# vvvwo/KSS-ICP

Measured on AMD Instinct MI355X. Metric: icp_iterations_per_sec, higher is better.
Workload: dtype f32; 1 GPU; C2: one 100000x100000 uniform-sphere pair per GPU, 50 fixed ICP iterations + fitness pass per step (exact NN + cov reduce + host 3x3 SVD), R_z(10deg), jitter 1e-3; n_src=100000, n_tgt=100000, pairs_per_gpu=1, nn_engine=cell list + brute-force fallback, nn_arithmetic=reference (no fma)

## Files before the change

kss-icp_amd/csrc/kss_api.hip:

```cpp
#pragma clang fp contract(off)

#include <cmath>

#include "kss_ctx.hpp"
#include "kss_gicp.hpp"
#include "kss_robust.hpp"

extern "C" {

int kss_version(void) { return KSS_VERSION; }

const char* kss_status_string(int s) {
    switch (s) {
        case KSS_OK: return "ok";
        case KSS_ERR_ARG: return "invalid argument";
        case KSS_ERR_HIP: return "HIP runtime error";
        case KSS_ERR_NOMEM: return "out of memory";
        case KSS_ERR_NODEVICE: return "no usable GPU device";
        case KSS_ERR_CAPACITY: return "output buffer too small";
        case KSS_ERR_RCCL: return "RCCL error";
        case KSS_ERR_DEGENERATE: return "degenerate point-to-plane system";
        default: return "unknown status";
    }
}

const char* kss_last_error(const kss_ctx* ctx) { return ctx ? ctx->err.c_str() : ""; }

static int ctx_create_common(int device_id, void* stream, bool borrow, kss_ctx** out) {
    if (!out) return KSS_ERR_ARG;
    *out = nullptr;
    int n = 0;
    if (hipGetDeviceCount(&n) != hipSuccess || n <= 0) return KSS_ERR_NODEVICE;
    if (device_id < 0 || device_id >= n) return KSS_ERR_ARG;
    if (hipSetDevice(device_id) != hipSuccess) return KSS_ERR_NODEVICE;
    kss_ctx* c = new (std::nothrow) kss_ctx();
    if (!c) return KSS_ERR_NOMEM;
    c->device = device_id;
    if (borrow) {
        c->stream = (hipStream_t)stream;
        c->own_stream = false;
    } else {
        if (hipStreamCreateWithFlags(&c->stream, hipStreamNonBlocking) != hipSuccess) { delete c; return KSS_ERR_HIP; }
        c->own_stream = true;
    }
    kss_live_contexts().fetch_add(1);
    static std::atomic<unsigned long long> ctx_serial{0};
    c->seq = (ctx_serial.fetch_add(1) + 1ull) << 40;
    *out = c;
    return KSS_OK;
}

int kss_ctx_create(int device_id, kss_ctx** out) { return ctx_create_common(device_id, nullptr, false, out); }
int kss_ctx_create_on_stream(int device_id, void* hip_stream, kss_ctx** out) {
    return ctx_create_common(device_id, hip_stream, true, out);
}

int kss_ctx_destroy(kss_ctx* c) {
    if (!c) return KSS_ERR_ARG;
    hipSetDevice(c->device);
    hipStreamSynchronize(c->stream);
    prof_collect(c);
    for (auto& ep : c->ev_pool) { hipEventDestroy(ep.a); hipEventDestroy(ep.b); }
    c->ev_pool.clear();
    DevBuf* bufs[] = {&c->tgt4, &c->src0, &c->cur[0], &c->cur[1], &c->keys, &c->partials, &c->sums, &c->nn_work,
                      &c->red_work, &c->pair_red, &c->state, &c->cs, &c->scratch_a, &c->scratch_b, &c->scratch_c,
                      &c->stage_src, &c->stage_tgt, &c->stage_idx, &c->stage_d2, &c->stage_out, &c->g_counts, &c->g_slot, &c->g_start,
                      &c->g_cursor, &c->g_bsums, &c->g_sorted, &c->g_list, &c->g_count, &c->g_bbox, &c->g_partials, &c->g_start2, &c->g_pairs, &c->g_stamps, &c->g_pos, &c->g_nnst, &c->res_pos, &c->res_wc, &c->res_perm, &c->pack_seg, &c->reg_s, &c->reg_t, &c->reg_p, &c->reg_all, &c->reg_f, &c->reg_g, &c->oct_pts, &c->oct_cen, &c->oct_a, &c->oct_b, &c->oct_tmp, &c->pre_partials, &c->pre_state, &c->g_rowpair, &c->g_gate, &c->p2l_idx, &c->p2l_d2, &c->p2l_perm, &c->p2l_rows, &c->p2l_nrm, &c->p2l_n64, &c->trim_rows, &c->trim_state, &c->rob_keys, &c->gicp_snrm, &c->pb_desc, &c->pb_rowpair, &c->pb_nrm, &c->pb_rscale, &c->pb_snrm, &c->pb_gicp, &c->o2o_table, &c->o2o_idx, &c->o2o_d2, &c->recip_sorted, &c->recip_box, &c->recip_grids, &c->gate_bar, &c->res_gate, &c->bar_state};
    for (DevBuf* b : bufs)
        if (b->p) hipFree(b->p);
    if (c->h_sums) hipHostFree(c->h_sums);
    if (c->h_seq) hipHostFree(c->h_seq);
    if (c->h_p2l) hipHostFree(c->h_p2l);
    if (c->h_gicp) hipHostFree(c->h_gicp);
    if (c->h_box) hipHostFree(c->h_box);
    if (c->h_xf) hipHostFree(c->h_xf);
    if (c->h_state) hipHostFree(c->h_state);
    for (kss_vmap* m : c->vmaps) { vmap_free(m->b); delete m; }
    c->vmaps.clear();
    for (kss_ctx* w : c->workers) kss_ctx_destroy(w);
    c->workers.clear();
    if (c->own_stream) hipStreamDestroy(c->stream);
    kss_live_contexts().fetch_sub(1);
    delete c;
    return KSS_OK;
}

int kss_ctx_synchronize(kss_ctx* c) {
    if (!c) return KSS_ERR_ARG;
    HIPCHK(c, hipStreamSynchronize(c->stream));
    return KSS_OK;
}

void* kss_ctx_stream(kss_ctx* c) { return c ? (void*)c->stream : nullptr; }

int kss_ctx_set_nn_mode(kss_ctx* c, int nn_mode) {
    if (!c || nn_mode < KSS_NN_AUTO || nn_mode > KSS_NN_GRID) return KSS_ERR_ARG;
    c->nn_mode = nn_mode;
    return KSS_OK;
}

int kss_profile_enable(kss_ctx* c, int on) {
    if (!c) return KSS_ERR_ARG;
    c->prof = on > 0 ? on : 0;
    for (int k = 0; k < KSS_K_COUNT; ++k) c->prof_tick[k] = 0;
    if (c->prof) {
        HIPCHK(c, hipSetDevice(c->device));
        while (c->ev_pool.size() < 4096) {
            kss_ctx::EvPair ep;
            if (hipEventCreate(&ep.a) != hipSuccess) break;
            if (hipEventCreate(&ep.b) != hipSuccess) { hipEventDestroy(ep.a); break; }
            c->ev_pool.push_back(ep);
        }
    }
    return KSS_OK;
}
int kss_grid_stats(kss_ctx* c, double out[8]) {
    if (!c || !out) return KSS_ERR_ARG;
    for (int k = 0; k < 8; ++k) out[k] = c->grid_stats[k];
    return KSS_OK;
}
int kss_debug_grid_evals(kss_ctx* c, double out[2]) {
    if (!c || !out) return KSS_ERR_ARG;
    out[0] = c->evals_sum; out[1] = c->evals_launches;
    c->evals_sum = 0.0; c->evals_launches = 0.0;
    return KSS_OK;
}

int kss_debug_grid_stamps(kss_ctx* c, unsigned long long* out, int64_t cap) {
    if (!c || !out) return KSS_ERR_ARG;
    if (c->stamps_nblk > 0 && c->g_stamps.p) {
        hipStreamSynchronize(c->stream);
        c->last_stamps.resize((size_t)c->stamps_nblk * 16);
        if (hipMemcpy(c->last_stamps.data(), (const unsigned long long*)c->g_stamps.p + (size_t)(c->stamps_seq & 1) * c->stamps_nblk * 16,
                      c->last_stamps.size() * sizeof(unsigned long long), hipMemcpyDeviceToHost) != hipSuccess) return KSS_ERR_HIP;
    }
    const int64_t n = std::min<int64_t>(cap, (int64_t)c->last_stamps.size());
    for (int64_t i = 0; i < n; ++i) out[i] = c->last_stamps[(size_t)i];
    return (int)n;
}
int kss_profile_reset(kss_ctx* c) {
    if (!c) return KSS_ERR_ARG;
    HIPCHK(c, hipStreamSynchronize(c->stream));
    prof_collect(c);
    for (int k = 0; k < KSS_K_COUNT; ++k) { c->prof_ms[k] = 0; c->prof_n[k] = 0; }
    return KSS_OK;
}
int kss_profile_event_overhead(kss_ctx* c, double* ms) {
    if (!c || !ms) return KSS_ERR_ARG;
    HIPCHK(c, hipSetDevice(c->device));
    hipEvent_t a = nullptr, b = nullptr;
    HIPCHK(c, hipEventCreate(&a));
    HIPCHK(c, hipEventCreate(&b));
    for (int i = 0; i < 16; ++i) launch_empty(c->stream);
    HIPCHK(c, hipStreamSynchronize(c->stream));
    double tot = 0.0;
    const int reps = 200;
    for (int i = 0; i < reps; ++i) {
        hipEventRecord(a, c->stream);
        launch_empty(c->stream);
        hipEventRecord(b, c->stream);
        HIPCHK(c, hipStreamSynchronize(c->stream));
        float e = 0.f;
        HIPCHK(c, hipEventElapsedTime(&e, a, b));
        tot += e;
    }
    hipEventDestroy(a);
    hipEventDestroy(b);
    *ms = tot / reps;
    return KSS_OK;
}
int kss_profile_get(kss_ctx* c, int k, double* total_ms, int64_t* launches) {
    if (!c || k < 0 || k >= KSS_K_COUNT) return KSS_ERR_ARG;
    HIPCHK(c, hipStreamSynchronize(c->stream));
    prof_collect(c);
    if (total_ms) *total_ms = c->prof_ms[k];
    if (launches) *launches = c->prof_n[k];
    return KSS_OK;
}

}

extern "C" {

int kss_icp_default_params(kss_icp_params* p) {
    if (!p) return KSS_ERR_ARG;
    std::memset(p, 0, sizeof *p);
    p->max_iterations = 1000;
    p->max_corr_dist = 1.0;
    p->transformation_epsilon = 1e-10;
    p->euclidean_fitness_epsilon = 0.001;
    p->abs_mse_epsilon = 1e-12;
    p->min_correspondences = 3;
    p->compute_fitness = 1;
    return KSS_OK;
}

int kss_icp_dev(kss_ctx* c, const float* d_src, int64_t ns, const float* d_tgt, int64_t nt,
                const kss_icp_params* p, kss_icp_result* res) {
    if (!c) return KSS_ERR_ARG;
    if (ns <= 0 || nt <= 0) return set_err(c, KSS_ERR_ARG, "icp: empty cloud");
    const int64_t so[2] = {0, ns}, to[2] = {0, nt};
    return icp_run_dev(c, d_src, so, d_tgt, to, 1, false, KSS_F32, p, res);
}

int kss_icp(kss_ctx* c, const float* src, int64_t ns, const float* tgt, int64_t nt,
            const kss_icp_params* p, kss_icp_result* res) {
    if (!c || !src || !tgt) return set_err(c, KSS_ERR_ARG, "icp: null cloud");
    if (ns <= 0 || nt <= 0) return set_err(c, KSS_ERR_ARG, "icp: empty cloud");
    HIPCHK(c, hipSetDevice(c->device));
    KCHK(upload(c, c->stage_src, src, (size_t)ns * 3 * sizeof(float)));
    KCHK(upload(c, c->stage_tgt, tgt, (size_t)nt * 3 * sizeof(float)));
    return kss_icp_dev(c, (const float*)c->stage_src.p, ns, (const float*)c->stage_tgt.p, nt, p, res);
}

int kss_icp_batch_dev(kss_ctx* c, const float* d_src_all, const int64_t* src_off, const float* d_tgt_all,
                      const int64_t* tgt_off, int npairs, const kss_icp_params* p, kss_icp_result* results) {
    if (!c) return KSS_ERR_ARG;
    return icp_run_dev(c, d_src_all, src_off, d_tgt_all, tgt_off, npairs, false, KSS_F32, p, results);
}

int kss_icp_batch(kss_ctx* c, const float* src_all, const int64_t* src_off, const float* tgt_all,
                  const int64_t* tgt_off, int npairs, const kss_icp_params* p, kss_icp_result* results) {
    if (!c || !src_all || !tgt_all || !src_off || !tgt_off || npairs <= 0) return set_err(c, KSS_ERR_ARG, "icp_batch: bad argument");
    HIPCHK(c, hipSetDevice(c->device));
    const int64_t s0 = src_off[0], s1 = src_off[npairs], t0 = tgt_off[0], t1 = tgt_off[npairs];
    if (s1 <= s0 || t1 <= t0) return set_err(c, KSS_ERR_ARG, "icp_batch: empty batch");
    KCHK(upload(c, c->stage_src, src_all + 3 * s0, (size_t)(s1 - s0) * 3 * sizeof(float)));
    KCHK(upload(c, c->stage_tgt, tgt_all + 3 * t0, (size_t)(t1 - t0) * 3 * sizeof(float)));
    std::vector<int64_t> so(npairs + 1), to(npairs + 1);
    for (int i = 0; i <= npairs; ++i) { so[i] = src_off[i] - s0; to[i] = tgt_off[i] - t0; }
    return icp_run_dev(c, c->stage_src.p, so.data(), c->stage_tgt.p, to.data(), npairs, false, KSS_F32, p, results);
}

int kss_nn_dev(kss_ctx* c, const float* d_src, int64_t ns, const float* d_tgt, int64_t nt, int32_t* d_idx, float* d_d2) {
    return nn_generic_dev(c, d_src, ns, d_tgt, nt, KSS_F32, d_idx, d_d2, nullptr);
}

int kss_nn(kss_ctx* c, const float* src, int64_t ns, const float* tgt, int64_t nt, int32_t* idx, float* d2) {
    if (!c || !src || !tgt) return set_err(c, KSS_ERR_ARG, "nn: null cloud");
    if (ns <= 0 || nt <= 0) return set_err(c, KSS_ERR_ARG, "nn: empty cloud");
    HIPCHK(c, hipSetDevice(c->device));
    KCHK(upload(c, c->stage_src, src, (size_t)ns * 3 * sizeof(float)));
    KCHK(upload(c, c->stage_tgt, tgt, (size_t)nt * 3 * sizeof(float)));
    KCHK(ensure(c, c->stage_idx, (size_t)ns * sizeof(int32_t)));
    KCHK(ensure(c, c->stage_d2, (size_t)ns * sizeof(float)));
    KCHK(kss_nn_dev(c, (const float*)c->stage_src.p, ns, (const float*)c->stage_tgt.p, nt, (int32_t*)c->stage_idx.p, (float*)c->stage_d2.p));
    if (idx) HIPCHK(c, hipMemcpyAsync(idx, c->stage_idx.p, (size_t)ns * sizeof(int32_t), hipMemcpyDeviceToHost, c->stream));
    if (d2) HIPCHK(c, hipMemcpyAsync(d2, c->stage_d2.p, (size_t)ns * sizeof(float), hipMemcpyDeviceToHost, c->stream));
    HIPCHK(c, hipStreamSynchronize(c->stream));
    return KSS_OK;
}

static int knn_generic_dev(kss_ctx* c, const void* d_q, int64_t nq, const void* d_t, int64_t nt, int dtype, int k, int32_t* d_idx, float* d_d2) {
    if (!c || !d_q || !d_t || !d_idx || !d_d2) return set_err(c, KSS_ERR_ARG, "knn: null argument");
    if (nq <= 0 || nt <= 0 || k < 1 || k > 64) return set_err(c, KSS_ERR_ARG, "knn: need nq, nt > 0 and 1 <= k <= 64");
    if (nq > 0x7fff0000ll || nt > 0x7fff0000ll) return set_err(c, KSS_ERR_ARG, "knn: cloud too large");
    HIPCHK(c, hipSetDevice(c->device));
    const int64_t nt_pad = (nt + NN_TILE - 1) / NN_TILE * NN_TILE;
    KCHK(ensure(c, c->tgt4, (size_t)nt_pad * sizeof(float4)));
    KCHK(ensure(c, c->src0, (size_t)nq * sizeof(float4)));
    if (dtype == KSS_F64) {
        launch_pack_f64_to_f4(c->stream, (const double*)d_q, nq, (float4*)c->src0.p, nq, false);
        launch_pack_f64_to_f4(c->stream, (const double*)d_t, nt, (float4*)c->tgt4.p, nt_pad, true);
    } else {
        launch_pack_f3_to_f4(c->stream, (const float*)d_q, nq, (float4*)c->src0.p, nq, false);
        launch_pack_f3_to_f4(c->stream, (const float*)d_t, nt, (float4*)c->tgt4.p, nt_pad, true);
    }
    size_t part_bytes = 0;
    const int n_split = knn_plan_splits((int)nq, (int)nt_pad, k, &part_bytes);
    if (part_bytes) KCHK(ensure(c, c->keys, part_bytes));
    {
        ProfScope ps(c, KSS_K_NN_SWEEP);
        launch_knn_sweep(c->stream, (const float4*)c->src0.p, (int)nq, (const float4*)c->tgt4.p, (int)nt_pad, k, d_idx, d_d2, n_split,
                         part_bytes ? c->keys.p : nullptr);
    }
    HIPCHK(c, hipGetLastError());
    return KSS_OK;
}

int kss_knn_dev(kss_ctx* c, const float* d_query, int64_t nq, const float* d_tgt, int64_t nt, int k, int32_t* d_idx, float* d_d2) {
    KCHK(knn_generic_dev(c, d_query, nq, d_tgt, nt, KSS_F32, k, d_idx, d_d2));
    HIPCHK(c, hipStreamSynchronize(c->stream));
    return KSS_OK;
}

int kss_knn(kss_ctx* c, const float* query, int64_t nq, const float* tgt, int64_t nt, int k, int32_t* idx, float* d2) {
    if (!c || !query || !tgt || !idx || !d2) return set_err(c, KSS_ERR_ARG, "knn: null argument");
    if (nq <= 0 || nt <= 0 || k < 1 || k > 64) return set_err(c, KSS_ERR_ARG, "knn: need nq, nt > 0 and 1 <= k <= 64");
    HIPCHK(c, hipSetDevice(c->device));
    KCHK(upload(c, c->stage_src, query, (size_t)nq * 3 * sizeof(float)));
    KCHK(upload(c, c->stage_tgt, tgt, (size_t)nt * 3 * sizeof(float)));
    KCHK(ensure(c, c->stage_idx, (size_t)nq * k * sizeof(int32_t)));
    KCHK(ensure(c, c->stage_d2, (size_t)nq * k * sizeof(float)));
    KCHK(knn_generic_dev(c, c->stage_src.p, nq, c->stage_tgt.p, nt, KSS_F32, k, (int32_t*)c->stage_idx.p, (float*)c->stage_d2.p));
    HIPCHK(c, hipMemcpyAsync(idx, c->stage_idx.p, (size_t)nq * k * sizeof(int32_t), hipMemcpyDeviceToHost, c->stream));
    HIPCHK(c, hipMemcpyAsync(d2, c->stage_d2.p, (size_t)nq * k * sizeof(float), hipMemcpyDeviceToHost, c->stream));
    HIPCHK(c, hipStreamSynchronize(c->stream));
    return KSS_OK;
}

int kss_normals(kss_ctx* c, const double* pts, int64_t n, int k, double* normals) {
    if (!c || !pts || !normals) return set_err(c, KSS_ERR_ARG, "normals: null argument");
    if (n <= 0 || k < 1 || k > 64) return set_err(c, KSS_ERR_ARG, "normals: need n > 0 and 1 <= k <= 64");
    if (k > n) k = (int)n;
    HIPCHK(c, hipSetDevice(c->device));
    KCHK(upload(c, c->scratch_a, pts, (size_t)n * 3 * sizeof(double)));
    KCHK(ensure(c, c->stage_idx, (size_t)n * k * sizeof(int32_t)));
    KCHK(ensure(c, c->stage_d2, (size_t)n * k * sizeof(float)));
    KCHK(ensure(c, c->stage_out, (size_t)n * 3 * sizeof(double)));
    KCHK(knn_generic_dev(c, c->scratch_a.p, n, c->scratch_a.p, n, KSS_F64, k, (int32_t*)c->stage_idx.p, (float*)c->stage_d2.p));
    launch_normals(c->stream, (const float4*)c->src0.p, (int)n, (const int32_t*)c->stage_idx.p, k, (double*)c->stage_out.p);
    HIPCHK(c, hipGetLastError());
    HIPCHK(c, hipMemcpyAsync(normals, c->stage_out.p, (size_t)n * 3 * sizeof(double), hipMemcpyDeviceToHost, c->stream));
    HIPCHK(c, hipStreamSynchronize(c->stream));
    return KSS_OK;
}

int kss_normals_orient(kss_ctx* c, const double* pts, int64_t n, double* normals) {
    if (!c || !pts || !normals) return set_err(c, KSS_ERR_ARG, "normals_orient: null argument");
    if (n <= 0 || n > 0x7fff0000ll) return set_err(c, KSS_ERR_ARG, "normals_orient: bad size");
    HIPCHK(c, hipSetDevice(c->device));
    const int Kn = 8;
    const int k = n < Kn ? (int)n : Kn;
    KCHK(upload(c, c->scratch_a, pts, (size_t)n * 3 * sizeof(double)));
    KCHK(ensure(c, c->stage_idx, (size_t)n * k * sizeof(int32_t)));
    KCHK(ensure(c, c->stage_d2, (size_t)n * k * sizeof(float)));
    KCHK(knn_generic_dev(c, c->scratch_a.p, n, c->scratch_a.p, n, KSS_F64, k, (int32_t*)c->stage_idx.p, (float*)c->stage_d2.p));
    std::vector<int32_t> ki((size_t)n * k);
    std::vector<float> kd((size_t)n * k);
    HIPCHK(c, hipMemcpyAsync(ki.data(), c->stage_idx.p, ki.size() * sizeof(int32_t), hipMemcpyDeviceToHost, c->stream));
    HIPCHK(c, hipMemcpyAsync(kd.data(), c->stage_d2.p, kd.size() * sizeof(float), hipMemcpyDeviceToHost, c->stream));
    HIPCHK(c, hipStreamSynchronize(c->stream));
    std::vector<char> judge((size_t)n, 0);
    std::vector<int64_t> listed((size_t)n, -1);
    std::vector<int32_t> cur(1, 0), nxt, par;
    judge[0] = 1;
    for (int64_t level = 0; !cur.empty(); ++level) {
        nxt.clear(); par.clear();
        for (const int32_t u : cur) {
            const size_t row = (size_t)u * k;
            const int first = kd[row] == 0 ? 1 : 0;
            for (int j = first; j < first + k - 1 && j < k; ++j) {
                const int32_t v = ki[row + j];
                if (judge[(size_t)v] || listed[(size_t)v] == level) continue;
                listed[(size_t)v] = level;
                nxt.push_back(v); par.push_back(u);
            }
        }
        for (size_t a = 0; a < nxt.size(); ++a) {
            const double* np_ = normals + 3 * (size_t)par[a];
            double* ns = normals + 3 * (size_t)nxt[a];
            double a1 = np_[0] * ns[0] + np_[1] * ns[1] + np_[2] * ns[2];
            double a2 = -np_[0] * ns[0] - np_[1] * ns[1] - np_[2] * ns[2];
            a1 = a1 > 1 ? 1 : (a1 < -1 ? -1 : a1);
            a2 = a2 > 1 ? 1 : (a2 < -1 ? -1 : a2);
            if (std::acos(a1) > std::acos(a2)) { ns[0] = -ns[0]; ns[1] = -ns[1]; ns[2] = -ns[2]; }
            judge[(size_t)nxt[a]] = 1;
        }
        cur.swap(nxt);
    }
    return KSS_OK;
}

int kss_cov_dev(kss_ctx* c, const float* d_src, const float* d_tgt, const int32_t* d_idx, int64_t n, int64_t nt,
                double max_d2, double sums[KSS_NSUMS]) {
    if (!c || !d_src || !d_tgt || !d_idx || !sums) return set_err(c, KSS_ERR_ARG, "cov: null argument");
    if (n <= 0 || nt <= 0) return set_err(c, KSS_ERR_ARG, "cov: empty input");
    HIPCHK(c, hipSetDevice(c->device));
    const int nb = stream_blocks(n);
    KCHK(ensure(c, c->partials, (size_t)nb * NSUMS * sizeof(double)));
    KCHK(ensure(c, c->sums, NSUMS * sizeof(double)));
    KCHK(ensure_pinned(c, c->h_sums, c->h_sums_cap, NSUMS * sizeof(double)));
    {
        ProfScope ps(c, KSS_K_CORR_REDUCE);
        launch_corr_reduce_idx(c->stream, d_src, d_tgt, d_idx, n, max_d2, (double*)c->partials.p, nb);
        launch_sum_columns(c->stream, (const double*)c->partials.p, nb, NSUMS, (double*)c->sums.p);
    }
    HIPCHK(c, hipGetLastError());
    HIPCHK(c, hipMemcpyAsync(c->h_sums, c->sums.p, NSUMS * sizeof(double), hipMemcpyDeviceToHost, c->stream));
    HIPCHK(c, hipStreamSynchronize(c->stream));
    std::memcpy(sums, c->h_sums, NSUMS * sizeof(double));
    return KSS_OK;
}

int kss_cov(kss_ctx* c, const float* src, const float* tgt, const int32_t* idx, int64_t n, int64_t nt, double max_d2,
            double sums[KSS_NSUMS]) {
    if (!c || !src || !tgt || !idx || !sums) return set_err(c, KSS_ERR_ARG, "cov: null argument");
    if (n <= 0 || nt <= 0) return set_err(c, KSS_ERR_ARG, "cov: empty input");
    for (int64_t i = 0; i < n; ++i)
        if (idx[i] < 0 || idx[i] >= nt) return set_err(c, KSS_ERR_ARG, "cov: index out of range");
    HIPCHK(c, hipSetDevice(c->device));
    KCHK(upload(c, c->stage_src, src, (size_t)n * 3 * sizeof(float)));
    KCHK(upload(c, c->stage_tgt, tgt, (size_t)nt * 3 * sizeof(float)));
    KCHK(upload(c, c->stage_idx, idx, (size_t)n * sizeof(int32_t)));
    return kss_cov_dev(c, (const float*)c->stage_src.p, (const float*)c->stage_tgt.p, (const int32_t*)c->stage_idx.p, n, nt, max_d2, sums);
}

int kss_rigid_from_sums(const double sums[KSS_NSUMS], float T[16]) {
    if (!sums || !T) return KSS_ERR_ARG;
    if (!(sums[0] >= 1.0)) return KSS_ERR_ARG;
    rigid_from_sums(sums, T);
    return KSS_OK;
}

static inline bool trim_overlap_ok(double overlap) { return overlap > 0.0 && overlap <= 1.0; }

struct PairClouds {
    const float* src = nullptr;
    const float* tgt = nullptr;
    const float* snrm = nullptr;
    const float* tnrm = nullptr;
    int64_t ns = 0, nt = 0;
    bool batch = false;
    const int64_t* src_off = nullptr;
    const int64_t* tgt_off = nullptr;
    int npairs = 1;
    std::vector<int64_t> so, to;
};
static PairClouds one_pair(const float* src, int64_t ns, const float* snrm, const float* tgt, int64_t nt, const float* tnrm) {
    PairClouds P;
    P.src = src; P.ns = ns; P.snrm = snrm; P.tgt = tgt; P.nt = nt; P.tnrm = tnrm;
    return P;
}
static PairClouds many_pairs(const float* src, const int64_t* src_off, const float* snrm, const float* tgt, const int64_t* tgt_off,
                             const float* tnrm, int npairs) {
    PairClouds P;
    P.src = src; P.src_off = src_off; P.snrm = snrm; P.tgt = tgt; P.tgt_off = tgt_off; P.tnrm = tnrm; P.npairs = npairs; P.batch = true;
// ... 1629 lines not shown
```

kss-icp_amd/csrc/kss_ctx.hpp:

```cpp
#pragma once
#include <dlfcn.h>
#include <hip/hip_runtime.h>

#include <algorithm>
#include <atomic>
#include <chrono>
#include <cmath>
#include <cstdio>
#include <cstdlib>
#include <cstring>
#include <mutex>
#include <string>
#include <thread>
#include <vector>

#include "kss_internal.hpp"
#include "kss_host_pool.hpp"

using namespace kss;

struct DevBuf {
    void* p = nullptr;
    size_t cap = 0;
};
struct BarBuf : DevBuf { bool failed = false; };

struct kss_vmap {
    kss_ctx* ctx = nullptr;
    VmapBuilt b;
    double leaf = 0.0;
    VmapDev dev() const { return VmapDev{b.cell, b.rec, {b.lo[0], b.lo[1], b.lo[2]}, b.inv, {b.dims[0], b.dims[1], b.dims[2]}}; }
};

struct kss_ctx {
    int device = 0;
    int cu_count = 0;
    hipStream_t stream = nullptr;
    bool own_stream = false;
    std::string err;
    int nn_mode = KSS_NN_AUTO;
    double grid_stats[8] = {0, 0, 0, 0, 0, 0, 0, 0};
    double last_setup_ms = 0, last_loop_ms = 0;
    double t_launch_us = 0, t_wait_us = 0, t_host_us = 0;
    bool timing = false;
    bool tables_staged = false;
    int64_t stats_ns = -1, stats_nt = -1;

    DevBuf tgt4, src0, cur[2], keys, partials, sums, nn_work, red_work, pair_red, state, cs, scratch_a,
        scratch_b, scratch_c, stage_src, stage_tgt, stage_idx, stage_d2, stage_out, g_counts, g_slot, g_start, g_cursor,
        g_bsums, g_sorted, g_list, g_count, g_bbox, g_partials, g_start2, g_pairs, g_stamps, g_pos, g_nnst, res_pos, res_wc, res_perm, pack_seg, reg_s, reg_t, reg_p, reg_all, reg_f, reg_g, oct_pts, oct_cen, oct_a, oct_b, oct_tmp, pre_partials, pre_state, g_rowpair, g_gate;
    DevBuf p2l_idx, p2l_d2, p2l_perm, p2l_rows, p2l_nrm, p2l_n64;
    DevBuf trim_rows, trim_state;
    DevBuf rob_keys;
    DevBuf gicp_snrm;
    DevBuf pb_desc, pb_rowpair, pb_nrm;
    DevBuf pb_rscale;
    DevBuf pb_snrm, pb_gicp;
    DevBuf o2o_table, o2o_idx, o2o_d2;
    DevBuf recip_sorted, recip_box, recip_grids;
    std::vector<RecipPairDev> h_recip_grids;
    int64_t recip_total_cells = 0;
    void* h_gicp = nullptr; size_t h_gicp_cap = 0;
    void* h_gicp_dev = nullptr;
    const PairState* last_state_dev = nullptr;
    HostPool pool;
    std::vector<kss_vmap*> vmaps;
    std::vector<kss_ctx*> workers;
    std::vector<unsigned long long> last_stamps;
    int stamps_nblk = 0; unsigned long long stamps_seq = 0;
    std::vector<float> h_bbox;
    unsigned int* h_box = nullptr; unsigned int* h_box_dev = nullptr; size_t h_box_bytes = 0;
    unsigned box_tag = 0; int box_rows = 0;
    double evals_sum = 0.0, evals_launches = 0.0;
    void* h_sums = nullptr;  size_t h_sums_cap = 0;
    void* h_sums_dev = nullptr;
    void* h_p2l = nullptr; size_t h_p2l_cap = 0;
    void* h_p2l_dev = nullptr;
    unsigned long long* h_seq = nullptr;
    unsigned long long* h_seq_dev = nullptr;
    size_t h_seq_bytes = 0;
    struct Gated {
        int supported = -1;
        bool want_next = false;
        bool pending = false;
        bool chain = false;
        int steps_left = 0;
        int max_steps = 1;
        int slot = 0;
        unsigned long long seq = 0;
        int32_t stamp = 0;
        const void* d_in = nullptr; void* d_out = nullptr;
        bool fma = false, full = false, want_full = false; double max_d2 = 0.0;
    } gated;
    bool ws_dirty = false;
    bool defer_wait = false;
    PairState* h_xf = nullptr; PairState* h_xf_dev = nullptr;
    bool fit_last = false;
    bool nn_have = false;
    BarBuf gate_bar, res_gate, bar_state;
    int large_bar = -1;
    unsigned res_launches = 0;
    double res_passes = 0.0;
    int cand_cap = 0, cand_cap_pad = -1, cand_cap_fma = -1;
    int spec_judge = -1; double spec_threshold = 0.0; bool spec_ran = false, spec_cancelled = false;
    std::chrono::steady_clock::time_point res_backoff[2] = {};
    unsigned long long seq = 0;
    void* h_state = nullptr; size_t h_state_cap = 0;

    int prof = 0;
    unsigned prof_tick[KSS_K_COUNT] = {};
    struct EvPair { hipEvent_t a, b; };
    std::vector<EvPair> ev[KSS_K_COUNT];
    std::vector<EvPair> ev_pool;
    double prof_ms[KSS_K_COUNT] = {0};
    int64_t prof_n[KSS_K_COUNT] = {0};
};

static inline int set_err(kss_ctx* c, int code, const char* what, hipError_t e = hipSuccess) {
    if (c) {
        c->err = what;
        if (e != hipSuccess) { c->err += ": "; c->err += hipGetErrorString(e); }
    }
    return code;
}

#define HIPCHK(ctx, call)                                                        \
    do {                                                                         \
        hipError_t e_ = (call);                                                  \
        if (e_ != hipSuccess) return set_err((ctx), KSS_ERR_HIP, #call, e_);     \
    } while (0)

static inline int ensure(kss_ctx* c, DevBuf& b, size_t bytes) {
    if (bytes <= b.cap) return KSS_OK;
    if (b.p) {
        HIPCHK(c, hipStreamSynchronize(c->stream));
        HIPCHK(c, hipFree(b.p));
        b.p = nullptr; b.cap = 0;
    }
    size_t want = bytes + bytes / 8 + 256;
    hipError_t e = hipMalloc(&b.p, want);
    if (e != hipSuccess) { b.p = nullptr; return set_err(c, KSS_ERR_NOMEM, "hipMalloc", e); }
    b.cap = want;
    return KSS_OK;
}

static inline int ensure_zeroed(kss_ctx* c, DevBuf& b, size_t bytes) {
    const size_t before = b.cap;
    const int rc = ensure(c, b, bytes);
    if (rc != KSS_OK) return rc;
    if (b.cap != before && hipMemsetAsync(b.p, 0, b.cap, c->stream) != hipSuccess) return set_err(c, KSS_ERR_HIP, "hipMemsetAsync(zero-at-rest buffer)");
    return KSS_OK;
}

inline void* bar_ensure(kss_ctx* c, BarBuf& b, size_t bytes) {
    static const bool want_bar = getenv("KSS_GATE_BAR") == nullptr || atoi(getenv("KSS_GATE_BAR")) != 0;
    if (!want_bar || b.failed) return nullptr;
    if (b.p && b.cap >= bytes) return b.p;
    hipDeviceProp_t prop;
    if (c->large_bar < 0) c->large_bar = hipGetDeviceProperties(&prop, c->device) == hipSuccess && prop.isLargeBar ? 1 : 0;
    if (b.p) { hipStreamSynchronize(c->stream); hipFree(b.p); b.p = nullptr; b.cap = 0; }
    const size_t cap = (bytes + bytes / 4 + 4095) / 4096 * 4096;
    void* p = nullptr;
    if (!c->large_bar || hipExtMallocWithFlags(&p, cap, hipDeviceMallocFinegrained) != hipSuccess || !p || hipMemset(p, 0, cap) != hipSuccess ||
        hipDeviceSynchronize() != hipSuccess) {
        (void)hipGetLastError();
        if (p) hipFree(p);
        b.failed = true;
        return nullptr;
    }
    b.p = p; b.cap = cap;
    return p;
}

static inline int ensure_pinned(kss_ctx* c, void*& p, size_t& cap, size_t bytes) {
    if (bytes <= cap) return KSS_OK;
    if (p) { HIPCHK(c, hipStreamSynchronize(c->stream)); HIPCHK(c, hipHostFree(p)); p = nullptr; cap = 0; }
    size_t want = bytes * 2 + 256;
    hipError_t e = hipHostMalloc(&p, want, hipHostMallocMapped);
    if (e != hipSuccess) { p = nullptr; return set_err(c, KSS_ERR_NOMEM, "hipHostMalloc", e); }
    cap = want;
    if (&p == &c->h_sums) {
        void* d = nullptr;
        HIPCHK(c, hipHostGetDevicePointer(&d, p, 0));
        c->h_sums_dev = d;
    }
    if (&p == &c->h_p2l) {
        void* d = nullptr;
        HIPCHK(c, hipHostGetDevicePointer(&d, p, 0));
        c->h_p2l_dev = d;
    }
    return KSS_OK;
}

#define KCHK(expr)                     \
    do {                               \
        int rc_ = (expr);              \
        if (rc_ != KSS_OK) return rc_; \
    } while (0)

struct ProfScope {
    kss_ctx* c; int k; kss_ctx::EvPair ep; bool on;
    ProfScope(kss_ctx* c_, int k_, bool every = false) : c(c_), k(k_), on(c_->prof > 0) {
        if (on && c->prof > 1 && !every) on = (c->prof_tick[k]++ % (unsigned)c->prof) == 0;
        if (!on) return;
        if (!c->ev_pool.empty()) {
            ep = c->ev_pool.back();
            c->ev_pool.pop_back();
        } else if (hipEventCreate(&ep.a) != hipSuccess || hipEventCreate(&ep.b) != hipSuccess) {
            on = false;
            return;
        }
        hipEventRecord(ep.a, c->stream);
    }
    ~ProfScope() {
        if (!on) return;
        hipEventRecord(ep.b, c->stream);
        c->ev[k].push_back(ep);
    }
};

static inline void prof_collect(kss_ctx* c) {
    for (int k = 0; k < KSS_K_COUNT; ++k) {
        for (auto& ep : c->ev[k]) {
            float ms = 0.f;
            if (hipEventElapsedTime(&ms, ep.a, ep.b) == hipSuccess) {
                c->prof_ms[k] += ms; c->prof_n[k] += 1;
                if (k == KSS_K_GRID_CHAIN) c->prof_ms[KSS_K_GRID_CHAIN_PASS] += ms;
                if (k == KSS_K_RESIDENT) c->prof_ms[KSS_K_RESIDENT_PASS] += ms;
            }
            c->ev_pool.push_back(ep);
        }
        c->ev[k].clear();
    }
}


inline std::atomic<int>& kss_live_contexts() { static std::atomic<int> n{0}; return n; }

static inline int upload(kss_ctx* c, DevBuf& b, const void* h, size_t bytes) {
    KCHK(ensure(c, b, bytes));
    HIPCHK(c, hipMemcpyAsync(b.p, h, bytes, hipMemcpyHostToDevice, c->stream));
    return KSS_OK;
}

namespace kss {
int icp_run_dev(kss_ctx* c, const void* d_src, const int64_t* src_off, const void* d_tgt, const int64_t* tgt_off,
                int npairs, bool shared_target, int dtype, const kss_icp_params* p, kss_icp_result* results);
int nn_generic_dev(kss_ctx* c, const void* d_src, int64_t ns, const void* d_tgt, int64_t nt, int dtype,
                   int32_t* d_idx, float* d_d2, double sums_out[NSUMS]);
struct PairMode {
    bool plane = false;
    bool trimmed = false;
    double overlap = 1.0;
    double* trace_info = nullptr;
    double* last_info = nullptr;
    bool robust = false;
    RobustScale rs;
    bool gicp = false;
    double gicp_epsilon = 0.0;
    const float* d_src_nrm = nullptr;
    bool symm = false;
    int symm_align = 1;
    bool sim = false;
    double scale_min = 1.0;
    double scale_max = 1.0;
    bool unique = false;
    bool mutual = false;
};
static_assert(KSS_ROBUST_NINFO == KSS_TRIM_NINFO, "the pair loop carries both info records in the same four slots");
int pair_run_dev(kss_ctx* c, const float* d_src, int64_t ns, const float* d_tgt, int64_t nt, const float* d_nrm,
                 const kss_icp_params* p, const PairMode& mode, kss_icp_result* res);
int pair_record_dev(kss_ctx* c, const float* d_src, const float* d_tgt, const float* d_nrm, const int32_t* d_idx, int64_t n, int64_t nt,
                    double max_d2, const PairMode& mode, const float* Rn, double* sums, double* info);
int trim_threshold_dev(kss_ctx* c, const float* d_d2, int64_t n, double max_d2, double overlap, double* info);
int vgicp_record_dev(kss_ctx* c, const float* d_src, const float* d_snrm, int64_t n, const kss_vmap* map, double max_d2, const float* Rn,
                     double epsilon, double* sums);
int vgicp_run_dev(kss_ctx* c, const float* d_src, int64_t ns, const float* d_snrm, const kss_vmap* map, const kss_icp_params* p, double epsilon,
                  kss_icp_result* res, double* info);
int pairs_run_dev(kss_ctx* c, const float* d_src, const int64_t* src_off, const float* d_tgt, const int64_t* tgt_off, const float* d_nrm,
                  int npairs, const kss_icp_params* p, const PairMode& mode, const double* overlaps, kss_icp_result* results, double* info_all,
                  const RobustScale* rscales = nullptr, const double* gicp_eps = nullptr, const int32_t* symm_aligns = nullptr);
int trim_threshold_batch_dev(kss_ctx* c, const float* d_d2, const int64_t* off, int nseg, double max_d2, const double* overlaps, double* info_all);
int o2o_filter_dev(kss_ctx* c, const int32_t* d_idx, const float* d_d2, const int64_t* off, const int64_t* nts, int nseg, double max_d2,
                   int32_t* d_idx_out, float* d_d2_out, double* info_all);
int recip_filter_dev(kss_ctx* c, const float* d_src, const int64_t* off, const float* d_tgt, const int64_t* tgt_off, int nseg,
                     const int32_t* d_idx, const float* d_d2, double max_d2, bool nn_fma, int32_t* d_idx_out, float* d_d2_out,
                     double* info_all, bool lone = false);
int ensure_pub_slots(kss_ctx* c);
int wait_slots(kss_ctx* c, int nslots, double* out);
}
```

kss-icp_amd/csrc/kss_engine.hip:

```cpp
#pragma clang fp contract(off)

#include <emmintrin.h>
#include <limits>

#include "kss_ctx.hpp"
#include "kss_pair_device.hpp"

namespace kss {

static int restore_zero_at_rest(kss_ctx* c);

static int resident_rows_limit(kss_ctx* c) {
    if (c->cu_count <= 0) {
        hipDeviceProp_t prop;
        c->cu_count = hipGetDeviceProperties(&prop, c->device) == hipSuccess && prop.multiProcessorCount > 0 ? prop.multiProcessorCount : 1;
        (void)hipGetLastError();
    }
    return c->cu_count;
}

constexpr int PUB_PAIRS = 32;
static int ensure_pub(kss_ctx* c, int npairs = PUB_PAIRS);

struct PairGeom {
    int64_t ns, nt;
    int32_t src_base;
    int32_t tgt_base;
    int32_t tgt_pad;
    int32_t n_split, chunk;
    int32_t key_base;
    int32_t n_src_blocks;
};

struct IcpPlan {
    int npairs = 0, S = 4;
    std::vector<PairGeom> g;
    mutable std::vector<NNWork> nn;
    int per_block = 0;
    size_t nn_count = 0;
    std::vector<RedWork> red;
    std::vector<PairRed> pred;
    int64_t total_src = 0, total_tgt_pad = 0, total_keys = 0;
    bool shared_target = false;
    bool grid = false;
    bool gridb = false;
    bool src_in_cell_order = false;
    GridParams gp;
    int total_cells = 0;
    std::vector<GridPairDev> gpairs;
    std::vector<int32_t> row_pair;
    int total_rows = 0;
};
constexpr int PASS_CHUNK = 512;

static void fill_nn_table(const IcpPlan& pl, int p) {
    const PairGeom& g = pl.g[p];
    const int per_block = pl.per_block;
    for (int b = 0; b < g.n_src_blocks; ++b)
        for (int s = 0; s < g.n_split; ++s) {
            NNWork w;
            w.pair = p;
            w.src_begin = g.src_base + b * per_block;
            w.src_count = (int32_t)std::min<int64_t>(per_block, g.ns - (int64_t)b * per_block);
            w.tgt_begin = g.tgt_base + s * g.chunk;
            w.tgt_count = g.chunk;
            w.tgt_pair_base = g.tgt_base;
            w.key_begin = g.key_base + (int32_t)((int64_t)s * g.ns) + b * per_block;
            w.write_src = s == 0;
            if (pl.grid) {
                w.src_begin = b * per_block;
                w.key_begin = g.key_base;
                w.write_src = g.src_base;
            }
            pl.nn.push_back(w);
        }
}

static int build_plan(kss_ctx* c, const int64_t* ns, const int64_t* nt, int npairs, bool shared_target,
               int S_req, int split_req, int nn_mode, IcpPlan& pl) {
    pl.npairs = npairs;
    pl.shared_target = shared_target;
    if (nn_mode == KSS_NN_AUTO) nn_mode = c->nn_mode;
    constexpr int64_t min_nt = 512, min_ns = 512;
    pl.grid = nn_mode == KSS_NN_GRID || (nn_mode == KSS_NN_AUTO && npairs == 1 && nt[0] >= min_nt && ns[0] >= min_ns);
    if (npairs != 1) pl.grid = false;
    if (npairs > 1 && !shared_target) {
        int64_t least_nt = nt[0], tot_ns = 0;
        for (int p = 0; p < npairs; ++p) { least_nt = std::min(least_nt, nt[p]); tot_ns += ns[p]; }
        pl.gridb = nn_mode == KSS_NN_GRID || (nn_mode == KSS_NN_AUTO && least_nt >= 2 * min_nt && tot_ns >= 32 * min_ns);
    }
    const bool any_grid = pl.grid || pl.gridb;
    pl.src_in_cell_order = any_grid;
    int64_t tot = 0;
    for (int p = 0; p < npairs; ++p) {
        if (ns[p] <= 0 || nt[p] <= 0) return set_err(c, KSS_ERR_ARG, "empty cloud in ICP pair");
        if (ns[p] > 0x7fff0000ll || nt[p] > 0x7fff0000ll) return set_err(c, KSS_ERR_ARG, "problem too large for 32-bit indexing");
        tot += ns[p];
    }
    int S = S_req;
    int64_t max_tiles = 1;
    for (int p = 0; p < npairs; ++p) max_tiles = std::max<int64_t>(max_tiles, (nt[p] + NN_TILE - 1) / NN_TILE);
    auto blocks_for = [&](int s) { int64_t b = 0; for (int p = 0; p < npairs; ++p) b += (ns[p] + (int64_t)NN_THREADS * s - 1) / ((int64_t)NN_THREADS * s); return b; };
    bool small = false;
    if (S != 1 && S != 2 && S != 4 && S != 8) {
        S = tot >= 32768 ? 4 : (tot >= 8192 ? 2 : 1);
        while (S > 1 && blocks_for(S) * max_tiles < 2048) S /= 2;
        small = blocks_for(S) * max_tiles < 2048;
    }
    pl.S = S;
    const int per_block = NN_THREADS * S;
    const int64_t src_blocks_total = blocks_for(S);
    int64_t want_split = 1;
    if (src_blocks_total < 2048) want_split = (4096 + src_blocks_total - 1) / src_blocks_total;
    if (split_req > 0) want_split = split_req;

    pl.g.resize(npairs);
    int64_t sb = 0, tb = 0, kb = 0;
    for (int p = 0; p < npairs; ++p) {
        PairGeom& g = pl.g[p];
        g.ns = ns[p]; g.nt = nt[p];
        const int64_t tiles = (nt[p] + NN_TILE - 1) / NN_TILE;
        int64_t split = std::min<int64_t>(want_split, std::max<int64_t>(1, small ? tiles : tiles / 2));
        int64_t chunk_tiles = (tiles + split - 1) / split;
        split = (tiles + chunk_tiles - 1) / chunk_tiles;
        g.n_split = (int32_t)split;
        g.chunk = (int32_t)(chunk_tiles * NN_TILE);
        g.tgt_pad = g.n_split * g.chunk;
        g.src_base = (int32_t)sb;
        g.key_base = (int32_t)kb;
        g.n_src_blocks = (int32_t)((ns[p] + per_block - 1) / per_block);
        if (shared_target && p > 0) {
            g.tgt_base = pl.g[0].tgt_base;
        } else {
            g.tgt_base = (int32_t)tb;
            tb += g.tgt_pad;
        }
        sb += ns[p];
        kb += any_grid ? ns[p] : (int64_t)g.n_split * ns[p];
        if (sb > 0x7fff0000ll || tb > 0x7fff0000ll || kb > 0x7fff0000ll)
            return set_err(c, KSS_ERR_ARG, "problem too large for 32-bit indexing");
    }
    pl.total_src = sb; pl.total_tgt_pad = tb; pl.total_keys = kb;
    pl.gpairs.clear(); pl.row_pair.clear(); pl.total_rows = 0;
    if (any_grid) {
        pl.gpairs.resize(npairs);
        for (int p = 0; p < npairs; ++p) {
            GridPairDev& gd = pl.gpairs[p];
            std::memset(&gd, 0, sizeof gd);
            gd.tgt_base = pl.g[p].tgt_base; gd.tgt_n = (int32_t)pl.g[p].nt; gd.tgt_pad = pl.g[p].tgt_pad;
            gd.src_base = pl.g[p].src_base; gd.src_n = (int32_t)pl.g[p].ns;
            gd.row_base = pl.total_rows;
            gd.n_rows = (int32_t)((pl.g[p].ns + PASS_CHUNK - 1) / PASS_CHUNK);
            for (int r = 0; r < gd.n_rows; ++r) pl.row_pair.push_back(p);
            pl.total_rows += gd.n_rows;
        }
    }

    pl.nn.clear(); pl.red.clear(); pl.pred.resize(npairs);
    pl.per_block = per_block;
    pl.nn_count = 0;
    int32_t prow = 0;
    for (int p = 0; p < npairs; ++p) {
        const PairGeom& g = pl.g[p];
        if (!pl.gridb) pl.nn_count += (size_t)g.n_src_blocks * g.n_split;
        if (!pl.gridb && !pl.grid) fill_nn_table(pl, p);
        pl.pred[p].first = prow;
        int64_t R = (g.ns + 256 * 512 - 1) / (256 * 512);
        R = std::max<int64_t>(1, std::min<int64_t>(R, 64));
        const int64_t rchunk = 256 * R;
        const int nrb = (pl.gridb || pl.grid) ? 0 : (int)((g.ns + rchunk - 1) / rchunk);
        for (int b = 0; b < nrb; ++b) {
            RedWork r;
            r.pair = p;
            r.src_begin = g.src_base + (int32_t)(b * rchunk);
            r.src_count = (int32_t)std::min<int64_t>(rchunk, g.ns - (int64_t)b * rchunk);
            r.key_begin = g.key_base + (int32_t)(b * rchunk);
            r.key_stride = (int32_t)g.ns;
            r.n_split = any_grid ? 1 : g.n_split;
            r.tgt_pair_base = g.tgt_base;
            r.partial_index = prow++;
            pl.red.push_back(r);
        }
        pl.pred[p].count = nrb;
    }
    return KSS_OK;
}

static int stage_tables(kss_ctx* c, const IcpPlan& pl) {
    if (c->tables_staged) return KSS_OK;
    if (pl.grid && pl.nn.empty())
        for (int p = 0; p < pl.npairs; ++p) fill_nn_table(pl, p);
    HIPCHK(c, hipMemcpyAsync(c->nn_work.p, pl.nn.data(), pl.nn.size() * sizeof(NNWork), hipMemcpyHostToDevice, c->stream));
    HIPCHK(c, hipMemcpyAsync(c->red_work.p, pl.red.data(), pl.red.size() * sizeof(RedWork), hipMemcpyHostToDevice, c->stream));
    HIPCHK(c, hipMemcpyAsync(c->pair_red.p, pl.pred.data(), pl.pred.size() * sizeof(PairRed), hipMemcpyHostToDevice, c->stream));
    HIPCHK(c, hipStreamSynchronize(c->stream));
    c->tables_staged = true;
    return KSS_OK;
}

static int stage_plan(kss_ctx* c, const IcpPlan& pl) {
    KCHK(ensure(c, c->tgt4, (size_t)pl.total_tgt_pad * sizeof(float4)));
    KCHK(ensure(c, c->src0, (size_t)pl.total_src * sizeof(float4)));
    KCHK(ensure(c, c->cur[0], (size_t)pl.total_src * sizeof(float4)));
    KCHK(ensure(c, c->cur[1], (size_t)pl.total_src * sizeof(float4)));
    KCHK(ensure(c, c->keys, (size_t)pl.total_keys * sizeof(unsigned long long)));
    KCHK(ensure_zeroed(c, c->partials, std::max<size_t>(pl.red.size(), (size_t)pl.total_rows) * NSUMS * sizeof(Granule)));
    KCHK(ensure(c, c->sums, (size_t)pl.npairs * NSUMS * sizeof(double)));
    KCHK(ensure(c, c->nn_work, pl.nn_count * sizeof(NNWork)));
    KCHK(ensure(c, c->red_work, pl.red.size() * sizeof(RedWork)));
    KCHK(ensure(c, c->pair_red, pl.pred.size() * sizeof(PairRed)));
    KCHK(ensure(c, c->state, (size_t)pl.npairs * sizeof(PairState)));
    KCHK(ensure_pinned(c, c->h_sums, c->h_sums_cap, (size_t)pl.npairs * NSUMS * sizeof(double)));
    KCHK(ensure_pinned(c, c->h_state, c->h_state_cap, (size_t)pl.npairs * sizeof(PairState)));
    KCHK(ensure_pub(c, pl.npairs));
    c->tables_staged = false;
    if (!pl.grid && !pl.shared_target) KCHK(stage_tables(c, pl));
    return KSS_OK;
}

static int pack_clouds(kss_ctx* c, const IcpPlan& pl, const void* d_src, const int64_t* src_off, const void* d_tgt,
                const int64_t* tgt_off, int dtype) {
    const size_t esz = dtype == KSS_F64 ? sizeof(double) : sizeof(float);
    if (pl.grid) {
        const PairGeom& g = pl.g[0];
        const int nbb = pack_pair_bbox_rows(g.tgt_pad);
        KCHK(ensure(c, c->g_bbox, (size_t)nbb * 6 * sizeof(float)));
        static const bool box_host = !(getenv("KSS_BBOX_HOST") && atoi(getenv("KSS_BBOX_HOST")) == 0);
        c->box_tag = 0; c->box_rows = 0;
        if (box_host && nbb <= 8192) {
            const size_t want = (size_t)nbb * 32;
            if (want > c->h_box_bytes) {
                if (c->h_box) { HIPCHK(c, hipStreamSynchronize(c->stream)); HIPCHK(c, hipHostFree(c->h_box)); c->h_box = nullptr; c->h_box_dev = nullptr; c->h_box_bytes = 0; }
                void* hp = nullptr; void* dp = nullptr;
                const size_t bytes = want + want / 2;
                if (hipHostMalloc(&hp, bytes, hipHostMallocMapped) == hipSuccess && hipHostGetDevicePointer(&dp, hp, 0) == hipSuccess) {
                    std::memset(hp, 0, bytes);
                    c->h_box = (unsigned int*)hp; c->h_box_dev = (unsigned int*)dp; c->h_box_bytes = bytes;
                } else { if (hp) hipHostFree(hp); (void)hipGetLastError(); }
            }
            if (c->h_box) {
                c->box_tag = (unsigned)(++c->seq);
                if (c->box_tag == 0) c->box_tag = (unsigned)(++c->seq);
                c->box_rows = nbb;
            }
        }
        launch_pack_pair(c->stream, dtype, (const char*)d_tgt + (size_t)tgt_off[0] * 3 * esz, g.nt, (float4*)c->tgt4.p + g.tgt_base, g.tgt_pad,
                         (float*)c->g_bbox.p, (const char*)d_src + (size_t)src_off[0] * 3 * esz, g.ns, (float4*)c->src0.p + g.src_base,
                         c->box_tag ? c->h_box_dev : nullptr, c->box_tag);
        HIPCHK(c, hipGetLastError());
        return KSS_OK;
    }
    {
        const char* base = (const char*)d_src + (size_t)src_off[0] * 3 * esz;
        if (dtype == KSS_F64) launch_pack_f64_to_f4(c->stream, (const double*)base, pl.total_src, (float4*)c->src0.p, pl.total_src, false);
        else launch_pack_f3_to_f4(c->stream, (const float*)base, pl.total_src, (float4*)c->src0.p, pl.total_src, false);
    }
    const int ntp = pl.shared_target ? 1 : pl.npairs;
    if (ntp > 8) {
        std::vector<PackSeg> seg((size_t)ntp);
        for (int p = 0; p < ntp; ++p) { seg[p].in_off = tgt_off[p]; seg[p].out_base = pl.g[p].tgt_base; seg[p].n = pl.g[p].nt; }
        KCHK(ensure(c, c->pack_seg, seg.size() * sizeof(PackSeg)));
        HIPCHK(c, hipMemcpyAsync(c->pack_seg.p, seg.data(), seg.size() * sizeof(PackSeg), hipMemcpyHostToDevice, c->stream));
        HIPCHK(c, hipStreamSynchronize(c->stream));
        launch_pack_batch(c->stream, d_tgt, dtype, (const PackSeg*)c->pack_seg.p, ntp, pl.total_tgt_pad, (float4*)c->tgt4.p);
        HIPCHK(c, hipGetLastError());
        return KSS_OK;
    }
    for (int p = 0; p < ntp; ++p) {
        const PairGeom& g = pl.g[p];
        const char* base = (const char*)d_tgt + (size_t)tgt_off[p] * 3 * esz;
        float4* out = (float4*)c->tgt4.p + g.tgt_base;
        if (dtype == KSS_F64) launch_pack_f64_to_f4(c->stream, (const double*)base, g.nt, out, g.tgt_pad, true);
        else launch_pack_f3_to_f4(c->stream, (const float*)base, g.nt, out, g.tgt_pad, true);
    }
    HIPCHK(c, hipGetLastError());
    return KSS_OK;
}

static void choose_cells(const float mn[3], const float mx[3], int64_t nt, GridParams& gp) {
    const float ext[3] = {mx[0] - mn[0], mx[1] - mn[1], mx[2] - mn[2]};
    const float emax = std::max(ext[0], std::max(ext[1], ext[2]));
    float hscale = 2.0f;
    if (const char* e = getenv("KSS_GRID_HSCALE")) { const float v = (float)atof(e); if (v > 0.05f && v < 50.f) hscale = v; }
    float h = emax * hscale * std::sqrt(3.0f / (float)nt);
    h = std::max(h, emax / 255.5f);
    if (!(h > 0.f)) h = 1.f;
    gp.ox = mn[0]; gp.oy = mn[1]; gp.oz = mn[2];
    gp.h = h; gp.inv_h = 1.0f / h;
    gp.gx = std::max(1, std::min(256, (int)std::floor(ext[0] / h) + 1));
    gp.gy = std::max(1, std::min(256, (int)std::floor(ext[1] / h) + 1));
    gp.gz = std::max(1, std::min(256, (int)std::floor(ext[2] / h) + 1));
    const float mag = std::max(std::max(std::fabs(mn[0]), std::fabs(mx[0])), std::max(std::max(std::fabs(mn[1]), std::fabs(mx[1])), std::max(std::fabs(mn[2]), std::fabs(mx[2]))));
    gp.eps = 2e-6f * (mag + emax) + 1e-30f;
    gp.rcap = 4;
}

static int grid_setup(kss_ctx* c, IcpPlan& pl) {
    if (!pl.grid) return KSS_OK;
    const PairGeom& g = pl.g[0];
    const int nt = (int)g.nt, ns = (int)g.ns;
    const int nbb = pack_pair_bbox_rows(g.tgt_pad);
    const float4* tgt = (const float4*)c->tgt4.p + g.tgt_base;
    ProfScope ps(c, KSS_K_GRID_BUILD);
    float mn[3] = {INFINITY, INFINITY, INFINITY}, mx[3] = {-INFINITY, -INFINITY, -INFINITY};
    bool have_box = false;
    if (c->box_tag != 0 && c->box_rows == nbb) {
        const unsigned long long* hq = (const unsigned long long*)c->h_box;
        const auto t0 = std::chrono::steady_clock::now();
        int g = 0;
        for (long spin = 0; g < 2 * nbb; ++spin) {
            const unsigned long long w0 = __atomic_load_n(&hq[2 * g], __ATOMIC_ACQUIRE), w1 = __atomic_load_n(&hq[2 * g + 1], __ATOMIC_ACQUIRE);
            const unsigned x = (unsigned)w0, y = (unsigned)(w0 >> 32), z = (unsigned)w1, tag = (unsigned)(w1 >> 32);
            if (tag - kss_mix3(x, y, z) == c->box_tag) {
                float f[3];
                std::memcpy(&f[0], &x, 4); std::memcpy(&f[1], &y, 4); std::memcpy(&f[2], &z, 4);
                for (int k = 0; k < 3; ++k) { if (g & 1) mx[k] = std::max(mx[k], f[k]); else mn[k] = std::min(mn[k], f[k]); }
                ++g;
                continue;
            }
            __builtin_ia32_pause();
            if ((spin & 4095) == 4095 && std::chrono::duration<double, std::milli>(std::chrono::steady_clock::now() - t0).count() > 20.0) break;
        }
        have_box = g == 2 * nbb;
        if (!have_box) { for (int k = 0; k < 3; ++k) { mn[k] = INFINITY; mx[k] = -INFINITY; } }
    }
    if (!have_box) {
        std::vector<float>& hb = c->h_bbox;
        hb.resize((size_t)nbb * 6);
        HIPCHK(c, hipMemcpyAsync(hb.data(), c->g_bbox.p, hb.size() * sizeof(float), hipMemcpyDeviceToHost, c->stream));
        HIPCHK(c, hipStreamSynchronize(c->stream));
        for (int b = 0; b < nbb; ++b)
            for (int k = 0; k < 3; ++k) { mn[k] = std::min(mn[k], hb[(size_t)b * 6 + k]); mx[k] = std::max(mx[k], hb[(size_t)b * 6 + 3 + k]); }
    }
    if (!(std::isfinite(mn[0]) && std::isfinite(mn[1]) && std::isfinite(mn[2]) && std::isfinite(mx[0]) && std::isfinite(mx[1]) && std::isfinite(mx[2])))
        return set_err(c, KSS_ERR_ARG, "non-finite target coordinates");
    GridParams gp;
    choose_cells(mn, mx, nt, gp);
    pl.gp = gp;
    const size_t ncells = (size_t)gp.gx * gp.gy * gp.gz;
    KCHK(ensure_zeroed(c, c->g_counts, 2 * ncells * sizeof(int32_t)));
    KCHK(ensure(c, c->g_slot, ((size_t)nt + (size_t)ns) * sizeof(int32_t)));
    KCHK(ensure(c, c->g_start, (2 * ncells + 8) * sizeof(int32_t)));
    KCHK(ensure(c, c->g_bsums, scan_scratch_bytes((int)(2 * ncells))));
    KCHK(ensure(c, c->g_sorted, (size_t)nt * sizeof(float4)));
    KCHK(ensure(c, c->g_list, (size_t)ns * sizeof(int32_t)));
    KCHK(ensure(c, c->g_pos, (size_t)ns * sizeof(float4)));
    c->nn_have = false;
    KCHK(ensure(c, c->g_nnst, (size_t)ns * sizeof(float2)));
    KCHK(ensure_zeroed(c, c->g_count, 64));
    if (getenv("KSS_COUNTS_CHECK")) {
        HIPCHK(c, hipStreamSynchronize(c->stream));
        std::vector<int32_t> h(2 * ncells);
        HIPCHK(c, hipMemcpy(h.data(), c->g_counts.p, h.size() * sizeof(int32_t), hipMemcpyDeviceToHost));
        size_t bad = 0, first = 0;
        for (size_t k = 0; k < h.size(); ++k)
            if (h[k] != 0) { if (!bad) first = k; ++bad; }
        if (bad) {
            std::fprintf(stderr, "[kss] counts check: %zu cells x 2 (%d x %d x %d), buffer %zu bytes, %zu non-zero counters, first at %zu = %d\n", ncells,
                         gp.gx, gp.gy, gp.gz, c->g_counts.cap, bad, first, h[first]);
            return set_err(c, KSS_ERR_HIP, "cell counters not zero at rest");
        }
    }
    pl.gpairs[0].gp = gp;
    pl.gpairs[0].cell_base = 0;
    launch_grid_build_pair(c->stream, tgt, nt, (float4*)c->src0.p + g.src_base, ns, gp, (int32_t*)c->g_counts.p, (int32_t*)c->g_slot.p,
                           (int32_t*)c->g_start.p + 1, (int32_t*)c->g_bsums.p, (float4*)c->g_sorted.p, (float4*)c->cur[0].p);
    HIPCHK(c, hipGetLastError());
    c->grid_stats[0] = gp.h; c->grid_stats[1] = gp.gx; c->grid_stats[2] = gp.gy; c->grid_stats[3] = gp.gz;
    if (c->stats_ns != ns || c->stats_nt != nt) { c->grid_stats[4] = 0; c->grid_stats[5] = 0; }
    c->grid_stats[6] = ns; c->grid_stats[7] = nt;
    if (c->prof && (c->stats_ns != ns || c->stats_nt != nt)) {
        c->stats_ns = ns; c->stats_nt = nt;
        KCHK(ensure(c, c->scratch_c, 64));
        HIPCHK(c, hipMemsetAsync(c->scratch_c.p, 0, 16, c->stream));
        launch_grid_stats(c->stream, (const float4*)c->src0.p + g.src_base, ns, gp, (const int32_t*)c->g_start.p + 1, (unsigned long long*)c->scratch_c.p);
        unsigned long long hst[2] = {0, 0};
        HIPCHK(c, hipMemcpyAsync(hst, c->scratch_c.p, 16, hipMemcpyDeviceToHost, c->stream));
        HIPCHK(c, hipStreamSynchronize(c->stream));
        c->grid_stats[5] = (double)hst[0];
        c->grid_stats[4] = (double)hst[1];
    }
    return KSS_OK;
}

static int grid_setup_batch(kss_ctx* c, IcpPlan& pl) {
    if (!pl.gridb) return KSS_OK;
    const int np = pl.npairs;
    std::vector<GridPairDev>& hp = pl.gpairs;
    int64_t sum_nt = 0;
    for (int p = 0; p < np; ++p) sum_nt += pl.g[p].nt;
    ProfScope ps(c, KSS_K_GRID_BUILD);
    KCHK(ensure(c, c->g_pairs, (size_t)np * sizeof(GridPairDev)));
    KCHK(ensure(c, c->g_bbox, (size_t)np * 6 * sizeof(float)));
    HIPCHK(c, hipMemcpyAsync(c->g_pairs.p, hp.data(), (size_t)np * sizeof(GridPairDev), hipMemcpyHostToDevice, c->stream));
    launch_gridb_bbox(c->stream, (const float4*)c->tgt4.p, (const GridPairDev*)c->g_pairs.p, np, (float*)c->g_bbox.p);
    std::vector<float> hb((size_t)np * 6);
    HIPCHK(c, hipMemcpyAsync(hb.data(), c->g_bbox.p, hb.size() * sizeof(float), hipMemcpyDeviceToHost, c->stream));
    HIPCHK(c, hipStreamSynchronize(c->stream));
    int64_t cells = 0, sorted_base = 0;
    int most_cells = 0;
    for (int p = 0; p < np; ++p) {
        const float* b = &hb[(size_t)p * 6];
        for (int k = 0; k < 6; ++k)
            if (!std::isfinite(b[k])) return set_err(c, KSS_ERR_ARG, "non-finite target coordinates");
        choose_cells(b, b + 3, pl.g[p].nt, hp[p].gp);
        hp[p].cell_base = (int32_t)cells;
        hp[p].sorted_base = (int32_t)sorted_base;
        const int64_t nc = (int64_t)hp[p].gp.gx * hp[p].gp.gy * hp[p].gp.gz;
        most_cells = (int)std::max<int64_t>(most_cells, nc);
        cells += nc;
        sorted_base += pl.g[p].nt;
        if (cells > 0x7fff0000ll) return set_err(c, KSS_ERR_ARG, "batch cell lists exceed 32-bit indexing");
    }
    pl.total_cells = (int)cells;
    HIPCHK(c, hipMemcpyAsync(c->g_pairs.p, hp.data(), (size_t)np * sizeof(GridPairDev), hipMemcpyHostToDevice, c->stream));
    KCHK(ensure(c, c->g_start, ((size_t)cells + 8) * sizeof(int32_t)));
    KCHK(ensure(c, c->g_sorted, (size_t)sum_nt * sizeof(float4)));
    KCHK(ensure(c, c->g_pos, (size_t)pl.total_src * sizeof(float4)));
    c->nn_have = false;
    KCHK(ensure(c, c->g_nnst, (size_t)pl.total_src * sizeof(float2)));
    KCHK(ensure(c, c->g_rowpair, pl.row_pair.size() * sizeof(int32_t)));
    HIPCHK(c, hipMemcpyAsync(c->g_rowpair.p, pl.row_pair.data(), pl.row_pair.size() * sizeof(int32_t), hipMemcpyHostToDevice, c->stream));
    bool half = true;
    for (int p = 0; p < np; ++p) half = half && pl.g[p].nt < 65536 && pl.g[p].ns < 65536;
    const bool built_in_lds = most_cells <= gridb_lds_max_cells(half) &&
        launch_gridb_build_lds(c->stream, (const float4*)c->tgt4.p, (float4*)c->src0.p, (float4*)c->cur[0].p, (const GridPairDev*)c->g_pairs.p, np,
                               (int32_t*)c->g_start.p + 1, (float4*)c->g_sorted.p, (int)most_cells, half);
    if (!built_in_lds) {
        KCHK(ensure_zeroed(c, c->g_counts, (size_t)cells * sizeof(int32_t)));
        KCHK(ensure(c, c->g_start2, ((size_t)cells + 1) * sizeof(int32_t)));
        KCHK(ensure(c, c->g_bsums, scan_scratch_bytes((int)cells)));
        if ((cells + 4095) / 4096 > 1024 * 16) return set_err(c, KSS_ERR_ARG, "batch cell lists too large for the scan");
        launch_gridb_build_targets(c->stream, (const float4*)c->tgt4.p, (int)pl.total_tgt_pad, (const GridPairDev*)c->g_pairs.p, np,
                                   (int)cells, (int32_t*)c->g_counts.p, (int32_t*)c->g_start.p + 1,
                                   (int32_t*)c->g_bsums.p, (float4*)c->g_sorted.p);
        launch_gridb_sort_sources(c->stream, (const float4*)c->src0.p, (int)pl.total_src, (const GridPairDev*)c->g_pairs.p, np, (int)cells,
                                  (int32_t*)c->g_counts.p, (int32_t*)c->g_start2.p, (int32_t*)c->g_bsums.p,
                                  (float4*)c->cur[0].p, (float4*)c->src0.p);
    }
    HIPCHK(c, hipGetLastError());
    HIPCHK(c, hipStreamSynchronize(c->stream));
    return KSS_OK;
}

static int ensure_pub(kss_ctx* c, int npairs) {
    const size_t want = (size_t)std::max(npairs, PUB_PAIRS) * (NSUMS + 1) * 16;
    if (c->h_seq && want <= c->h_seq_bytes) return KSS_OK;
    if (c->h_seq) {
        HIPCHK(c, hipStreamSynchronize(c->stream));
        HIPCHK(c, hipHostFree(c->h_seq));
        c->h_seq = nullptr; c->h_seq_dev = nullptr; c->h_seq_bytes = 0;
    }
    void* p = nullptr;
    const size_t bytes = want + want / 4;
    if (hipHostMalloc(&p, bytes, hipHostMallocMapped) != hipSuccess) return set_err(c, KSS_ERR_NOMEM, "hipHostMalloc(result slots)");
    c->h_seq = (unsigned long long*)p;
    c->h_seq_bytes = bytes;
    std::memset(p, 0, bytes);
    void* d = nullptr;
    HIPCHK(c, hipHostGetDevicePointer(&d, p, 0));
    c->h_seq_dev = (unsigned long long*)d;
    return KSS_OK;
}

static void gated_cancel(kss_ctx* c);

static inline bool collect_pair(kss_ctx* c, int p, unsigned long long want) {
    const unsigned long long* sl = c->h_seq + (size_t)2 * NSUMS * p;
    double* out = (double*)c->h_sums + (size_t)NSUMS * p;
    if (!slots_collect(sl + 2 * (NSUMS - 1), 1, want, out + NSUMS - 1)) return false;
    return slots_collect(sl, NSUMS, want, out);
}

static int wait_pair(kss_ctx* c, int p, unsigned long long want) {
    for (long spin = 0; spin < 2000000; ++spin) {
        if (collect_pair(c, p, want)) return KSS_OK;
        __builtin_ia32_pause();
    }
    return KSS_ERR_HIP;
}

static int wait_seq(kss_ctx* c, int npairs = 1, unsigned long long want = 0, const int* active = nullptr, bool* not_published = nullptr) {
    if (!want) want = c->seq;
    bool slow = false;
    for (int p = npairs - 1; p >= 0; --p) {
        if (active && !active[p]) continue;
        if (!slow && wait_pair(c, p, want) == KSS_OK) continue;
        if (!slow) {
            gated_cancel(c);
            HIPCHK(c, hipStreamSynchronize(c->stream));
            slow = true;
        }
        if (!collect_pair(c, p, want)) {
            if (not_published) *not_published = true;
            return set_err(c, KSS_ERR_HIP, "kernel finished without publishing its result");
        }
    }
    return KSS_OK;
}

int ensure_pub_slots(kss_ctx* c) { return ensure_pub(c); }
int wait_slots(kss_ctx* c, int nslots, double* out) {
    const unsigned long long want = c->seq;
    for (long spin = 0; spin < 2000000; ++spin) {
        if (slots_collect(c->h_seq, nslots, want, out)) return KSS_OK;
        __builtin_ia32_pause();
    }
    HIPCHK(c, hipStreamSynchronize(c->stream));
    if (!slots_collect(c->h_seq, nslots, want, out)) return set_err(c, KSS_ERR_HIP, "kernel finished without publishing its result");
    return KSS_OK;
}

static bool gated_available(kss_ctx* c) {
    static const bool want = getenv("KSS_GATED") == nullptr || atoi(getenv("KSS_GATED")) != 0;
    if (!want || !c->own_stream || kss_live_contexts().load() != 1) return false;
    if (c->gated.supported < 0) {
        c->gated.supported = 0;
        if (bar_ensure(c, c->gate_bar, 256)) {
            c->gated.supported = 1;
            return true;
        }
        void *x = nullptr, *xd = nullptr;
        if (ensure(c, c->g_gate, 256) == KSS_OK && hipMemsetAsync(c->g_gate.p, 0, 256, c->stream) == hipSuccess &&
            hipHostMalloc(&x, 2 * sizeof(PairState), hipHostMallocMapped) == hipSuccess && hipHostGetDevicePointer(&xd, x, 0) == hipSuccess) {
            std::memset(x, 0, 2 * sizeof(PairState));
            c->h_xf = (PairState*)x; c->h_xf_dev = (PairState*)xd;
            c->gated.supported = 1;
        } else {
            (void)hipGetLastError();
            if (x) hipHostFree(x);
        }
    }
    return c->gated.supported == 1;
}

static void gated_release(kss_ctx* c, const PairState& st, int skip) {
    if (c->gate_bar.p) {
        unsigned words[16];
        std::memcpy(words, &st, sizeof st);
        words[14] = (unsigned)skip;
        static const long torn_at = getenv("KSS_TEST_TORN_GATE") ? atol(getenv("KSS_TEST_TORN_GATE")) : -1;
        static long released = 0;
        gate_record_store((unsigned*)c->gate_bar.p + 32 * c->gated.slot, words, (unsigned)c->gated.stamp, ++released == torn_at);
    } else {
        PairState* rec = &c->h_xf[c->gated.slot];
        for (int k = 0; k < 12; ++k) rec->m[k] = st.m[k];
        rec->active = st.active; rec->apply = st.apply; rec->pad[0] = skip;
        __atomic_store_n(&rec->pad[1], c->gated.stamp, __ATOMIC_RELEASE);
    }
    kss_ctx::Gated& G = c->gated;
    if (!skip && --G.steps_left > 0) {
        G.slot ^= 1;
        G.stamp += 1;
        G.seq += 1;
        const void* in = G.d_out; G.d_out = const_cast<void*>(G.d_in); G.d_in = in;
    } else {
        G.pending = false;
        G.steps_left = 0;
    }
}

static void gated_cancel(kss_ctx* c) {
    if (!c->gated.pending) return;
    PairState none;
    std::memset(&none, 0, sizeof none);
    gated_release(c, none, 1);
}

struct GatedGuard {
    kss_ctx* c;
    explicit GatedGuard(kss_ctx* c_) : c(c_) {}
    ~GatedGuard() { gated_cancel(c); c->gated.want_next = false; }
};

static float skin_setting() {
    static const float skin = getenv("KSS_SKIN") ? (float)atof(getenv("KSS_SKIN")) : 0.25f;
    return skin;
}
static int gate_polls_setting() {
    static const int gate_polls = getenv("KSS_GATE_POLLS") ? atoi(getenv("KSS_GATE_POLLS")) : (1 << 22);
    return gate_polls;
}

static PassArgs pass_args(kss_ctx* c, const IcpPlan& pl, const float4* d_in, float4* d_out, double max_d2,
                          int32_t* d_idx_out, float* d_d2_out) {
    PassArgs a;
    std::memset(&a, 0, sizeof a);
    a.src_in = d_in; a.src_out = d_out;
    a.cell_start = (const int32_t*)c->g_start.p + 1;
    a.sorted = (const float4*)c->g_sorted.p;
    a.tgt4 = (const float4*)c->tgt4.p;
    a.nn_win = (float4*)c->g_pos.p;
    a.nn_state = (float2*)c->g_nnst.p;
    a.skin = skin_setting();
    a.chain_len = 1;
    a.gate_polls = gate_polls_setting();
    a.chained = d_in != (const float4*)c->src0.p ? 1 : c->fit_last ? 2 : 0;
    a.src_last0 = (const float4*)c->cur[0].p; a.src_last1 = (const float4*)c->cur[1].p;
    a.keys = (unsigned long long*)c->keys.p;
    a.list = (int32_t*)c->g_list.p; a.list_count = (int32_t*)c->g_count.p;
    a.total_rows = pl.total_rows;
    a.use_prev = c->nn_have ? 1 : 0;
    a.max_d2 = max_d2;
    a.rows = (Granule*)c->partials.p;
    a.pub = c->h_seq_dev;
    a.idx_out = d_idx_out; a.d2_out = d_d2_out;
    {
        static const long torn_at = getenv("KSS_TEST_TORN_SLOT") ? atol(getenv("KSS_TEST_TORN_SLOT")) : -1;
        static long launches = 0;
        a.test_torn = torn_at > 0 && ++launches == torn_at ? 1 : 0;
    }
    if (pl.gridb) {
        a.pairs = (const GridPairDev*)c->g_pairs.p;
        a.row_pair = (const int32_t*)c->g_rowpair.p;
        a.defer_pairs = pl.npairs > resident_rows_limit(c) ? pl.npairs : 0;
    } else {
        a.pair0 = pl.gpairs[0];
    }
    return a;
}

struct GridPass {
    const IcpPlan& pl;
    bool fma, full;
    const float4* d_in; float4* d_out;
    double max_d2;
    int32_t* d_idx_out; float* d_d2_out;
    PassArgs a;
    int nblk;
    unsigned long long* stamps2 = nullptr;
    bool plain_args = false;
    unsigned long long want_seq = 0;
    bool via_gate = false;
};

static void grid_launch_plain(kss_ctx* c, GridPass& g) {
    ProfScope ps(c, KSS_K_GRID_NN);
    g.a.ps0 = ((const PairState*)c->h_state)[0];
    g.a.seq = ++c->seq;
    if (g.stamps2) g.a.stamps = g.stamps2 + (size_t)(g.a.seq & 1) * g.nblk * 16;
    launch_grid_pass(c->stream, g.fma, g.full, false, true, g.a);
    c->nn_have = true;
    g.want_seq = c->seq;
}

static void grid_release_or_launch(kss_ctx* c, GridPass& g) {
    kss_ctx::Gated& G = c->gated;
    if (G.pending && G.d_in == (const void*)g.d_in && G.d_out == (void*)g.d_out && G.fma == g.fma && G.full == g.full && G.max_d2 == g.max_d2 && g.plain_args) {
        g.want_seq = G.seq;
        c->seq = std::max(c->seq, G.seq);
        if (G.chain && c->prof > 0) c->prof_n[KSS_K_GRID_CHAIN_PASS] += 1;
        g.via_gate = true;
        static const long drop_at = getenv("KSS_TEST_DROP_GATE") ? atol(getenv("KSS_TEST_DROP_GATE")) : -1;
        static long releases = 0;
        if (++releases == drop_at) { G.pending = false; G.steps_left = 0; }
        else gated_release(c, ((const PairState*)c->h_state)[0], 0);
    } else {
        gated_cancel(c);
        grid_launch_plain(c, g);
    }
}

static void grid_enqueue_next(kss_ctx* c, const GridPass& g) {
    kss_ctx::Gated& G = c->gated;
    const bool next_sampled = c->prof == 1 || (c->prof > 1 && c->prof_tick[KSS_K_GRID_NN] % (unsigned)c->prof == 0);
    static const bool want_chain = getenv("KSS_CHAIN") == nullptr || atoi(getenv("KSS_CHAIN")) != 0;
    int len = 1;
    if (G.want_next && !G.pending && g.plain_args && gated_available(c) && want_chain && c->gate_bar.p &&
        (g.pl.total_rows <= resident_rows_limit(c) || g.pl.total_rows == 1))
        len = std::max(1, std::min(G.max_steps, 1 << 16));
    if (!(G.want_next && !G.pending && g.plain_args && gated_available(c) && (len > 1 || !next_sampled))) return;
    if (c->prof > 1 && len == 1) ++c->prof_tick[KSS_K_GRID_NN];
    float4* nxt_out = g.d_out == (float4*)c->cur[0].p ? (float4*)c->cur[1].p : (float4*)c->cur[0].p;
    G.slot ^= 1;
    G.stamp = (G.stamp + 1) & 0x7fffffff;
    if (G.stamp == 0 || G.stamp > 0x7fffffff - len - 1) G.stamp = 1;
    PassArgs n = pass_args(c, g.pl, g.d_out, nxt_out, g.max_d2, nullptr, nullptr);
    n.ps0 = ((const PairState*)c->h_state)[0];
    n.gate_seq = G.stamp;
    if (c->gate_bar.p) {
        n.state = nullptr;
        n.gate_dev = (unsigned int*)c->gate_bar.p;
        n.gate_slot = G.slot;
        n.chain_len = len;
        n.src_alt = g.d_out;
    } else {
        n.state = c->h_xf_dev + G.slot;
        n.gate_dev = (unsigned int*)c->g_gate.p;
    }
    n.seq = c->seq + 1;
    if (g.stamps2) n.stamps = g.stamps2 + (size_t)(n.seq & 1) * g.nblk * 16;
    if (len > 1) {
        ProfScope ps(c, KSS_K_GRID_CHAIN, true);
        launch_grid_pass(c->stream, g.fma, G.want_full, false, true, n);
    } else {
        launch_grid_pass(c->stream, g.fma, G.want_full, false, true, n);
    }
    G.chain = len > 1;
    G.pending = true; G.steps_left = len; G.seq = n.seq; G.d_in = g.d_out; G.d_out = nxt_out; G.fma = g.fma; G.full = G.want_full; G.max_d2 = g.max_d2;
    if (hipGetLastError() != hipSuccess) { gated_cancel(c); G.supported = 0; }
}

static int grid_wait(kss_ctx* c, GridPass& g) {
    bool not_published = false;
    const int rcw = wait_seq(c, 1, g.want_seq, nullptr, &not_published);
    if (rcw == KSS_OK || !g.via_gate || !not_published) return rcw;
    c->gated.pending = false; c->gated.steps_left = 0;
    c->err.clear();
// ... 1506 lines not shown
```

kss-icp_amd/csrc/kss_grid.hip:

```cpp
#pragma clang fp contract(off)

#include <hip/hip_runtime.h>

#include <cstring>

#include <rocprim/rocprim.hpp>

#include <cstdlib>

#include "kss_internal.hpp"
#include "kss_device.hpp"

namespace kss {

__global__ __launch_bounds__(256) void grid_count2_kernel(const float4* __restrict__ tgt, int nt, int nbt, const float4* __restrict__ src, int ns,
                                                          GridParams gp, int32_t* __restrict__ counts, int32_t* __restrict__ slot) {
    const bool is_src = (int)blockIdx.x >= nbt;
    const int i = ((int)blockIdx.x - (is_src ? nbt : 0)) * 256 + (int)threadIdx.x;
    if (i >= (is_src ? ns : nt)) return;
    const float4 p = is_src ? src[i] : tgt[i];
    const int cx = cell_coord(p.x, gp.ox, gp.inv_h, gp.gx), cy = cell_coord(p.y, gp.oy, gp.inv_h, gp.gy),
              cz = cell_coord(p.z, gp.oz, gp.inv_h, gp.gz);
    slot[(is_src ? nt : 0) + i] = atomicAdd(&counts[(is_src ? gp.gx * gp.gy * gp.gz : 0) + (cz * gp.gy + cy) * gp.gx + cx], 1);
}

constexpr int SCAN_CHUNK = 4096;

__global__ __launch_bounds__(256) void scan_block_sums_kernel(const int32_t* __restrict__ in, int n, int32_t* __restrict__ block_sums) {
    __shared__ int sh[4];
    typedef int32_t int4u __attribute__((ext_vector_type(4), aligned(4)));
    const int base = blockIdx.x * SCAN_CHUNK;
    int s = 0;
#pragma unroll
    for (int k = 0; k < 4; ++k) {
        const int i = base + (k * 256 + (int)threadIdx.x) * 4;
        if (i + 3 < n) { const int4u v = *(const int4u*)(in + i); s += (v.x + v.y) + (v.z + v.w); }
        else { if (i < n) s += in[i]; if (i + 1 < n) s += in[i + 1]; if (i + 2 < n) s += in[i + 2]; }
    }
#pragma unroll
    for (int off = 32; off > 0; off >>= 1) s += __shfl_down(s, off, 64);
    if ((threadIdx.x & 63) == 0) sh[threadIdx.x >> 6] = s;
    __syncthreads();
    if (threadIdx.x == 0) block_sums[blockIdx.x] = sh[0] + sh[1] + sh[2] + sh[3];
}

__global__ __launch_bounds__(1024) void scan_of_block_sums_kernel(int32_t* __restrict__ block_sums, int nb) {
    __shared__ int wave_tot[16];
    const int tid = threadIdx.x, lane = tid & 63, wave = tid >> 6;
    const int per = (nb + 1023) / 1024;
    const int lo = min(tid * per, nb), hi = min(nb, lo + per);
    int s = 0;
    for (int i = lo; i < hi; ++i) s += block_sums[i];
    int incl = s;
#pragma unroll
    for (int off = 1; off < 64; off <<= 1) {
        const int v = __shfl_up(incl, off, 64);
        if (lane >= off) incl += v;
    }
    if (lane == 63) wave_tot[wave] = incl;
    __syncthreads();
    int run = incl - s;
    for (int w = 0; w < 16; ++w) run += w < wave ? wave_tot[w] : 0;
    for (int i = lo; i < hi; ++i) {
        const int v = block_sums[i];
        block_sums[i] = run;
        run += v;
    }
}

template <bool SELF, bool CLEAR>
__global__ __launch_bounds__(256) void scan_apply_kernel(int32_t* in, int n, const int32_t* __restrict__ block_sums,
                                                         int32_t* __restrict__ out_start) {
    typedef int32_t int4u __attribute__((ext_vector_type(4), aligned(4)));
    __shared__ int sh_tot[4][4];
    __shared__ int sh_off[4];
    const int tid = threadIdx.x, lane = tid & 63, wave = tid >> 6;
    int offset = 0;
    if constexpr (SELF) {
        int part = 0;
        for (int b = tid; b < (int)blockIdx.x; b += 256) part += block_sums[b];
#pragma unroll
        for (int off = 32; off > 0; off >>= 1) part += __shfl_down(part, off, 64);
        if (lane == 0) sh_off[wave] = part;
    } else {
        offset = block_sums[blockIdx.x];
    }
    const int base = blockIdx.x * SCAN_CHUNK;
    int4u v[4];
    int incl[4];
#pragma unroll
    for (int k = 0; k < 4; ++k) {
        const int i = base + (k * 256 + tid) * 4;
        if (i + 3 < n) v[k] = *(const int4u*)(in + i);
        else { v[k].x = i < n ? in[i] : 0; v[k].y = i + 1 < n ? in[i + 1] : 0; v[k].z = i + 2 < n ? in[i + 2] : 0; v[k].w = 0; }
        if constexpr (CLEAR) {
            if (i + 3 < n) { if ((v[k].x | v[k].y | v[k].z | v[k].w) != 0) *(int4u*)(in + i) = int4u{0, 0, 0, 0}; }
            else { if (i < n) in[i] = 0; if (i + 1 < n) in[i + 1] = 0; if (i + 2 < n) in[i + 2] = 0; }
        }
        int x = (v[k].x + v[k].y) + (v[k].z + v[k].w);
#pragma unroll
        for (int off = 1; off < 64; off <<= 1) {
            const int t = __shfl_up(x, off, 64);
            if (lane >= off) x += t;
        }
        incl[k] = x;
        if (lane == 63) sh_tot[k][wave] = x;
    }
    __syncthreads();
    if constexpr (SELF) offset = sh_off[0] + sh_off[1] + sh_off[2] + sh_off[3];
    int run = offset;
#pragma unroll
    for (int k = 0; k < 4; ++k) {
        int before = 0;
#pragma unroll
        for (int w = 0; w < 4; ++w) before += w < wave ? sh_tot[k][w] : 0;
        const int own = (v[k].x + v[k].y) + (v[k].z + v[k].w);
        const int r0 = run + before + (incl[k] - own);
        const int i = base + (k * 256 + tid) * 4;
        int4u o;
        o.x = r0; o.y = r0 + v[k].x; o.z = o.y + v[k].y; o.w = o.z + v[k].z;
        if (i + 3 < n) *(int4u*)(out_start + i) = o;
        else { if (i < n) out_start[i] = o.x; if (i + 1 < n) out_start[i + 1] = o.y; if (i + 2 < n) out_start[i + 2] = o.z; }
        if (i <= n - 1 && n - 1 <= i + 3) out_start[n] = o.x + (n - 1 >= i ? v[k].x : 0) + (n - 1 >= i + 1 ? v[k].y : 0) + (n - 1 >= i + 2 ? v[k].z : 0) + (n - 1 >= i + 3 ? v[k].w : 0);
        run += (sh_tot[k][0] + sh_tot[k][1]) + (sh_tot[k][2] + sh_tot[k][3]);
    }
}

using BigScanConfig = rocprim::scan_config<256, 64, rocprim::block_load_method::block_load_transpose, rocprim::block_store_method::block_store_transpose,
                                           rocprim::block_scan_algorithm::reduce_then_scan>;

size_t scan_scratch_bytes(int n) {
    size_t bytes = 0;
    if (rocprim::inclusive_scan<BigScanConfig>(nullptr, bytes, (const int32_t*)nullptr, (int32_t*)nullptr, (size_t)n, rocprim::plus<int32_t>(), (hipStream_t)0) != hipSuccess) bytes = 0;
    return std::max<size_t>(bytes, ((size_t)(n + SCAN_CHUNK - 1) / SCAN_CHUNK + 1) * sizeof(int32_t)) + 256;
}

void launch_scan(hipStream_t st, int32_t* d_counts, int ncells, int32_t* d_start, int32_t* d_scratch, bool clear) {
    static const bool lib = getenv("KSS_SCAN_LIB") != nullptr;
    if (lib && ncells > 1024 * SCAN_CHUNK) {
        size_t bytes = 0;
        if (rocprim::inclusive_scan<BigScanConfig>(nullptr, bytes, d_counts, d_start + 1, (size_t)ncells, rocprim::plus<int32_t>(), st) == hipSuccess) {
            hipMemsetAsync(d_start, 0, sizeof(int32_t), st);
            if (rocprim::inclusive_scan<BigScanConfig>((void*)d_scratch, bytes, d_counts, d_start + 1, (size_t)ncells, rocprim::plus<int32_t>(), st) == hipSuccess) {
                if (clear) hipMemsetAsync(d_counts, 0, sizeof(int32_t) * (size_t)ncells, st);
                return;
            }
        }
        (void)hipGetLastError();
    }
    int32_t* d_block_sums = d_scratch;
    const int nb = (ncells + SCAN_CHUNK - 1) / SCAN_CHUNK;
    hipLaunchKernelGGL(scan_block_sums_kernel, dim3(nb), dim3(256), 0, st, (const int32_t*)d_counts, ncells, d_block_sums);
    if (nb <= 1024) {
        if (clear) hipLaunchKernelGGL((scan_apply_kernel<true, true>), dim3(nb), dim3(256), 0, st, d_counts, ncells, (const int32_t*)d_block_sums, d_start);
        else hipLaunchKernelGGL((scan_apply_kernel<true, false>), dim3(nb), dim3(256), 0, st, d_counts, ncells, (const int32_t*)d_block_sums, d_start);
    } else {
        hipLaunchKernelGGL(scan_of_block_sums_kernel, dim3(1), dim3(1024), 0, st, d_block_sums, nb);
        if (clear) hipLaunchKernelGGL((scan_apply_kernel<false, true>), dim3(nb), dim3(256), 0, st, d_counts, ncells, (const int32_t*)d_block_sums, d_start);
        else hipLaunchKernelGGL((scan_apply_kernel<false, false>), dim3(nb), dim3(256), 0, st, d_counts, ncells, (const int32_t*)d_block_sums, d_start);
    }
}

__global__ __launch_bounds__(256) void grid_scatter2_kernel(const float4* __restrict__ tgt, int nt, int nbt, const float4* __restrict__ src, int ns,
                                                            GridParams gp, const int32_t* __restrict__ slot, const int32_t* __restrict__ start,
                                                            float4* __restrict__ sorted, float4* __restrict__ src_tmp) {
    const bool is_src = (int)blockIdx.x >= nbt;
    const int i = ((int)blockIdx.x - (is_src ? nbt : 0)) * 256 + (int)threadIdx.x;
    if (i >= (is_src ? ns : nt)) return;
    float4 p = is_src ? src[i] : tgt[i];
    const int cx = cell_coord(p.x, gp.ox, gp.inv_h, gp.gx), cy = cell_coord(p.y, gp.oy, gp.inv_h, gp.gy),
              cz = cell_coord(p.z, gp.oz, gp.inv_h, gp.gz);
    const int cell = (is_src ? gp.gx * gp.gy * gp.gz : 0) + (cz * gp.gy + cy) * gp.gx + cx;
    const int pos = start[cell] + slot[(is_src ? nt : 0) + i] - (is_src ? nt : 0);
    p.w = __int_as_float(i);
    (is_src ? src_tmp : sorted)[pos] = p;
}

template <bool FMA>
__device__ __forceinline__ unsigned long long point_key(const float4 p, float qx, float qy, float qz) {
    const float dx = qx - p.x, dy = qy - p.y, dz = qz - p.z;
    float d;
    if constexpr (FMA) d = __builtin_fmaf(dx, dx, __builtin_fmaf(dy, dy, dz * dz));
    else d = (dx * dx + dy * dy) + dz * dz;
    return ((unsigned long long)__float_as_uint(d) << 32) | (unsigned long long)(unsigned)__float_as_int(p.w);
}

template <bool FMA>
__device__ __forceinline__ void scan_range(const float4* __restrict__ sorted, int lo, int hi, float qx, float qy, float qz,
                                           unsigned long long& key, int& kpos) {
    for (int k = lo; k < hi; k += 4) {
        const int k1 = min(k + 1, hi - 1), k2 = min(k + 2, hi - 1), k3 = min(k + 3, hi - 1);
        const float4 p0 = sorted[k], p1 = sorted[k1], p2 = sorted[k2], p3 = sorted[k3];
        const unsigned long long e0 = point_key<FMA>(p0, qx, qy, qz), e1 = point_key<FMA>(p1, qx, qy, qz),
                                 e2 = point_key<FMA>(p2, qx, qy, qz), e3 = point_key<FMA>(p3, qx, qy, qz);
        if (e0 < key) { key = e0; kpos = k; }
        if (e1 < key) { key = e1; kpos = k1; }
        if (e2 < key) { key = e2; kpos = k2; }
        if (e3 < key) { key = e3; kpos = k3; }
    }
}

typedef int32_t int4u __attribute__((ext_vector_type(4), aligned(4)));

template <bool FMA, int BS, int U>
__device__ __forceinline__ int block_walk(const GridParams& gp, const int32_t* __restrict__ cell_start, const float4* __restrict__ sorted,
                                          float qx, float qy, float qz, int cx, int cy, int cz, float rho, unsigned rowmask,
                                          int2 (*rowq)[BS], unsigned long long& key, int& kpos, float& m1, float& m2) {
    int s0[9], s1[9], s2[9], s3[9];
    bool ok[9];
#pragma unroll
    for (int t = 0; t < 9; ++t) {
        const int z = cz + t / 3 - 1, y = cy + t % 3 - 1;
        ok[t] = z >= 0 && z < gp.gz && y >= 0 && y < gp.gy && ((rowmask >> t) & 1u) != 0u;
        const int row = ok[t] ? (z * gp.gy + y) * gp.gx : 0;
        const int4u v = *(const int4u*)(cell_start + row + cx - 1);
        s0[t] = cx > 0 ? v.x : v.y;
        s1[t] = v.y;
        s2[t] = v.z;
        s3[t] = cx + 1 < gp.gx ? v.w : v.z;
    }
    const float exl = fmaxf((qx - (gp.ox + (float)cx * gp.h)) - gp.eps, 0.f), exr = fmaxf(((gp.ox + (float)(cx + 1) * gp.h) - qx) - gp.eps, 0.f);
    const float eyl = fmaxf((qy - (gp.oy + (float)cy * gp.h)) - gp.eps, 0.f), eyr = fmaxf(((gp.oy + (float)(cy + 1) * gp.h) - qy) - gp.eps, 0.f);
    const float ezl = fmaxf((qz - (gp.oz + (float)cz * gp.h)) - gp.eps, 0.f), ezr = fmaxf(((gp.oz + (float)(cz + 1) * gp.h) - qz) - gp.eps, 0.f);
    const float exl2 = exl * exl, exr2 = exr * exr;
    const float ey2[3] = {eyl * eyl, 0.f, eyr * eyr}, ez2[3] = {ezl * ezl, 0.f, ezr * ezr};
    int nrow = 0, total = 0;
#pragma unroll
    for (int t = 0; t < 9; ++t) {
        const float g2 = ey2[t % 3] + ez2[t / 3];
        const bool need = ok[t] && !(rho < g2 * 0.999999f);
        const bool left = !(rho < (g2 + exl2) * 0.999999f), right = !(rho < (g2 + exr2) * 0.999999f);
        const int lo = left ? s0[t] : s1[t];
        const int hi = right ? s3[t] : s2[t];
        const bool take = need && hi > lo;
        rowq[min(nrow, 8)][threadIdx.x] = make_int2(lo, hi);
        nrow += take ? 1 : 0;
        total += take ? hi - lo : 0;
    }
    int cur = 0, end = 0, nxt = 0;
    if (nrow > 0) { const int2 v = rowq[0][threadIdx.x]; cur = v.x; end = v.y; nxt = 1; }
    m1 = __builtin_inff();
    m2 = __builtin_inff();
    for (int e = 0; e < total; e += U) {
        int at[U];
#pragma unroll
        for (int j = 0; j < U; ++j) {
            at[j] = min(cur, end - 1);
            ++cur;
            if (cur >= end && nxt < nrow) { const int2 v = rowq[nxt][threadIdx.x]; cur = v.x; end = v.y; ++nxt; }
        }
        float4 pt[U];
#pragma unroll
        for (int j = 0; j < U; ++j) pt[j] = sorted[at[j]];
#pragma unroll
        for (int j = 0; j < U; ++j) {
            const unsigned long long kk = point_key<FMA>(pt[j], qx, qy, qz);
            if (kk < key) { key = kk; kpos = at[j]; }
            const float dd = e + j < total ? __uint_as_float((unsigned)(kk >> 32)) : __builtin_inff();
            m2 = __builtin_amdgcn_fmed3f(m1, m2, dd);
            m1 = fminf(m1, dd);
        }
    }
    return total;
}

#ifndef KSS_FIRST_U1
#define KSS_FIRST_U1 16
#endif
template <bool FMA, int BS, int U>
__device__ __forceinline__ int block_walk_first(const GridParams& gp, const int32_t* __restrict__ cell_start, const float4* __restrict__ sorted,
                                                float qx, float qy, float qz, int cx, int cy, int cz, float& rho, float skin,
                                                int2 (*rowq)[BS], unsigned long long& key, int& kpos, float& m1, float& m2) {
    constexpr int U1 = KSS_FIRST_U1;
    int s0[9], s1[9], s2[9], s3[9];
    bool ok[9];
#pragma unroll
    for (int t = 0; t < 9; ++t) {
        const int z = cz + t / 3 - 1, y = cy + t % 3 - 1;
        ok[t] = z >= 0 && z < gp.gz && y >= 0 && y < gp.gy;
        const int row = ok[t] ? (z * gp.gy + y) * gp.gx : 0;
        const int4u v = *(const int4u*)(cell_start + row + cx - 1);
        s0[t] = cx > 0 ? v.x : v.y;
        s1[t] = v.y;
        s2[t] = v.z;
        s3[t] = cx + 1 < gp.gx ? v.w : v.z;
    }
    m1 = __builtin_inff();
    m2 = __builtin_inff();
    const int lo4 = s0[4], n4 = s3[4] - s0[4];
    for (int e = 0; e < n4; e += U1) {
        int at[U1];
        float4 pt[U1];
#pragma unroll
        for (int j = 0; j < U1; ++j) at[j] = lo4 + min(e + j, n4 - 1);
#pragma unroll
        for (int j = 0; j < U1; ++j) pt[j] = sorted[at[j]];
#pragma unroll
        for (int j = 0; j < U1; ++j) {
            const unsigned long long kk = point_key<FMA>(pt[j], qx, qy, qz);
            if (kk < key) { key = kk; kpos = at[j]; }
            const float dd = e + j < n4 ? __uint_as_float((unsigned)(kk >> 32)) : __builtin_inff();
            m2 = __builtin_amdgcn_fmed3f(m1, m2, dd);
            m1 = fminf(m1, dd);
        }
    }
    if (rho == __builtin_inff() && key != ~0ull) {
        const float d0 = __uint_as_float((unsigned)(key >> 32));
        const float grown = __builtin_amdgcn_sqrtf(d0) + fmaxf(skin, 0.f) * gp.h;
        rho = skin >= 0.f ? fmaxf(d0, grown * grown) : d0;
    }
    const float exl = fmaxf((qx - (gp.ox + (float)cx * gp.h)) - gp.eps, 0.f), exr = fmaxf(((gp.ox + (float)(cx + 1) * gp.h) - qx) - gp.eps, 0.f);
    const float eyl = fmaxf((qy - (gp.oy + (float)cy * gp.h)) - gp.eps, 0.f), eyr = fmaxf(((gp.oy + (float)(cy + 1) * gp.h) - qy) - gp.eps, 0.f);
    const float ezl = fmaxf((qz - (gp.oz + (float)cz * gp.h)) - gp.eps, 0.f), ezr = fmaxf(((gp.oz + (float)(cz + 1) * gp.h) - qz) - gp.eps, 0.f);
    const float exl2 = exl * exl, exr2 = exr * exr;
    const float ey2[3] = {eyl * eyl, 0.f, eyr * eyr}, ez2[3] = {ezl * ezl, 0.f, ezr * ezr};
    int nrow = 0, total = 0;
#pragma unroll
    for (int t = 0; t < 9; ++t) {
        if (t == 4) continue;
        const float g2 = ey2[t % 3] + ez2[t / 3];
        const bool need = ok[t] && !(rho < g2 * 0.999999f);
        const bool left = !(rho < (g2 + exl2) * 0.999999f), right = !(rho < (g2 + exr2) * 0.999999f);
        const int lo = left ? s0[t] : s1[t];
        const int hi = right ? s3[t] : s2[t];
        const bool take = need && hi > lo;
        rowq[min(nrow, 7)][threadIdx.x] = make_int2(lo, hi);
        nrow += take ? 1 : 0;
        total += take ? hi - lo : 0;
    }
    int cur = 0, end = 0, nxt = 0;
    if (nrow > 0) { const int2 v = rowq[0][threadIdx.x]; cur = v.x; end = v.y; nxt = 1; }
    for (int e = 0; e < total; e += U) {
        int at[U];
#pragma unroll
        for (int j = 0; j < U; ++j) {
            at[j] = min(cur, end - 1);
            ++cur;
            if (cur >= end && nxt < nrow) { const int2 v = rowq[nxt][threadIdx.x]; cur = v.x; end = v.y; ++nxt; }
        }
        float4 pt[U];
#pragma unroll
        for (int j = 0; j < U; ++j) pt[j] = sorted[at[j]];
#pragma unroll
        for (int j = 0; j < U; ++j) {
            const unsigned long long kk = point_key<FMA>(pt[j], qx, qy, qz);
            if (kk < key) { key = kk; kpos = at[j]; }
            const float dd = e + j < total ? __uint_as_float((unsigned)(kk >> 32)) : __builtin_inff();
            m2 = __builtin_amdgcn_fmed3f(m1, m2, dd);
            m1 = fminf(m1, dd);
        }
    }
    return n4 + total;
}

__device__ __forceinline__ void row_range(const GridParams& gp, const int32_t* __restrict__ cell_start, float qx, float qy, float qz,
                                          int cx, int cy, int cz, float rho, int t, int& lo, int& hi) {
    lo = hi = 0;
    const int tz = t / 3, ty = t - 3 * tz;
    const int z = cz + tz - 1, y = cy + ty - 1;
    if (!(t >= 0 && t < 9 && z >= 0 && z < gp.gz && y >= 0 && y < gp.gy)) return;
    const int4u v = *(const int4u*)(cell_start + (z * gp.gy + y) * gp.gx + cx - 1);
    const int s0 = cx > 0 ? v.x : v.y, s1 = v.y, s2 = v.z, s3 = cx + 1 < gp.gx ? v.w : v.z;
    const float exl = fmaxf((qx - (gp.ox + (float)cx * gp.h)) - gp.eps, 0.f), exr = fmaxf(((gp.ox + (float)(cx + 1) * gp.h) - qx) - gp.eps, 0.f);
    const float eyl = fmaxf((qy - (gp.oy + (float)cy * gp.h)) - gp.eps, 0.f), eyr = fmaxf(((gp.oy + (float)(cy + 1) * gp.h) - qy) - gp.eps, 0.f);
    const float ezl = fmaxf((qz - (gp.oz + (float)cz * gp.h)) - gp.eps, 0.f), ezr = fmaxf(((gp.oz + (float)(cz + 1) * gp.h) - qz) - gp.eps, 0.f);
    const float ey2 = ty == 0 ? eyl * eyl : ty == 2 ? eyr * eyr : 0.f, ez2 = tz == 0 ? ezl * ezl : tz == 2 ? ezr * ezr : 0.f;
    const float g2 = ey2 + ez2;
    if (rho < g2 * 0.999999f) return;
    const bool left = !(rho < (g2 + exl * exl) * 0.999999f), right = !(rho < (g2 + exr * exr) * 0.999999f);
    lo = left ? s0 : s1;
    hi = right ? s3 : s2;
    if (hi < lo) hi = lo;
}

template <bool FMA, int U, bool TWO>
__device__ __forceinline__ void row_walk(const GridParams& gp, const int32_t* __restrict__ cell_start, const float4* __restrict__ sorted,
                                         float qx, float qy, float qz, int cx, int cy, int cz, float rho, int t0, int t1,
                                         unsigned long long& key, int& kpos, float& m1, float& m2) {
    m1 = __builtin_inff();
    m2 = __builtin_inff();
    int lo0, hi0, lo1 = 0, hi1 = 0;
    row_range(gp, cell_start, qx, qy, qz, cx, cy, cz, rho, t0, lo0, hi0);
    if constexpr (TWO) row_range(gp, cell_start, qx, qy, qz, cx, cy, cz, rho, t1, lo1, hi1);
    const int n0 = hi0 - lo0, total = n0 + (hi1 - lo1);
    const int last = hi1 > lo1 ? hi1 - 1 : hi0 - 1;
    for (int e = 0; e < total; e += U) {
        int at[U];
        float4 pt[U];
#pragma unroll
        for (int j = 0; j < U; ++j) {
            const int f = e + j;
            if constexpr (TWO) at[j] = f >= total ? last : f < n0 ? lo0 + f : lo1 + (f - n0);
            else at[j] = min(lo0 + f, hi0 - 1);
        }
#pragma unroll
        for (int j = 0; j < U; ++j) pt[j] = sorted[at[j]];
#pragma unroll
        for (int j = 0; j < U; ++j) {
            const unsigned long long kk = point_key<FMA>(pt[j], qx, qy, qz);
            if (kk < key) { key = kk; kpos = at[j]; }
            const float dd = e + j < total ? __uint_as_float((unsigned)(kk >> 32)) : __builtin_inff();
            m2 = __builtin_amdgcn_fmed3f(m1, m2, dd);
            m1 = fminf(m1, dd);
        }
    }
}

__global__ __launch_bounds__(256) void grid_rank_fix_kernel(const float4* __restrict__ tmp, int n, GridParams gp,
                                                            const int32_t* __restrict__ start , int shift,
                                                            float4* __restrict__ out) {
    const int j = blockIdx.x * blockDim.x + threadIdx.x;
    if (j >= n) return;
    const float4 p = tmp[j];
    const int cx = cell_coord(p.x, gp.ox, gp.inv_h, gp.gx), cy = cell_coord(p.y, gp.oy, gp.inv_h, gp.gy),
              cz = cell_coord(p.z, gp.oz, gp.inv_h, gp.gz);
    const int c = (cz * gp.gy + cy) * gp.gx + cx;
    const int lo = start[c] - shift, hi = start[c + 1] - shift;
    const int me = __float_as_int(p.w);
    int rank = 0;
    for (int k = lo; k < hi; ++k) rank += __float_as_int(tmp[k].w) < me ? 1 : 0;
    out[lo + rank] = p;
}

void launch_grid_build_pair(hipStream_t st, const float4* d_tgt, int nt, float4* d_src, int ns, const GridParams& gp, int32_t* d_counts,
                            int32_t* d_slot, int32_t* d_start, int32_t* d_block_sums, float4* d_sorted, float4* d_tmp) {
    const int ncells = gp.gx * gp.gy * gp.gz;
    const int nbt = (nt + 255) / 256, nbs = (ns + 255) / 256;
    hipLaunchKernelGGL(grid_count2_kernel, dim3(nbt + nbs), dim3(256), 0, st, d_tgt, nt, nbt, (const float4*)d_src, ns, gp, d_counts, d_slot);
    launch_scan(st, d_counts, 2 * ncells, d_start, d_block_sums, true);
    hipLaunchKernelGGL(grid_scatter2_kernel, dim3(nbt + nbs), dim3(256), 0, st, d_tgt, nt, nbt, (const float4*)d_src, ns, gp, (const int32_t*)d_slot,
                       (const int32_t*)d_start, d_sorted, d_tmp);
    hipLaunchKernelGGL(grid_rank_fix_kernel, dim3(nbs), dim3(256), 0, st, (const float4*)d_tmp, ns, gp, (const int32_t*)d_start + ncells, nt,
                       d_src);
}

struct SkipOut {
    unsigned long long key;
    int kpos;
    float rho;
    float acc;
    bool walker;
};
template <bool FMA>
__device__ __forceinline__ SkipOut skip_test(bool qok, float qx, float qy, float qz, float pold_x, float pold_y, float pold_z, const float4& prevp,
                                             const float2& st, bool chained_k, float skin_frac, float h) {
    SkipOut o;
    o.key = ~0ull; o.kpos = -1; o.rho = __builtin_inff(); o.acc = 0.f; o.walker = false;
    if (!qok) return o;
    o.walker = true;
    if (__float_as_uint(prevp.w) != ~0u) {
        o.key = point_key<FMA>(prevp, qx, qy, qz);
        o.kpos = -2;
        const float d0 = __uint_as_float((unsigned)(o.key >> 32));
        const float mx = qx - pold_x, my = qy - pold_y, mz = qz - pold_z;
        const float moved = __builtin_amdgcn_sqrtf((mx * mx + my * my) + mz * mz);
        const float acc = (st.y + moved) * 1.00001f;
        const float room = st.x - acc;
        if (chained_k && skin_frac >= 0.f && room > 1e-7f && (room * room) * 0.99999f > d0) {
            o.walker = false;
            o.acc = acc;
        } else {
            const float skin = fmaxf(skin_frac, 0.f) * h, grown = __builtin_amdgcn_sqrtf(d0) + skin;
            o.rho = !chained_k || moved * 4.f <= skin ? fmaxf(d0, grown * grown) : d0;
        }
    }
    return o;
}

template <bool FULL>
__device__ __forceinline__ void wave_row(bool have, bool kept, bool fell_back, float qx, float qy, float qz, const float4& win, double d2d, double* shw_row) {
    const int lane = threadIdx.x & 63;
    double col[16];
    {
        const double px = kept ? (double)qx : 0.0, py = kept ? (double)qy : 0.0, pz = kept ? (double)qz : 0.0;
        const double tx = kept ? (double)win.x : 0.0, ty = kept ? (double)win.y : 0.0, tz = kept ? (double)win.z : 0.0;
        col[0] = px; col[1] = py; col[2] = pz; col[3] = tx; col[4] = ty; col[5] = tz;
        col[6] = px * tx; col[7] = px * ty; col[8] = px * tz;
        col[9] = py * tx; col[10] = py * ty; col[11] = py * tz;
        col[12] = pz * tx; col[13] = pz * ty; col[14] = pz * tz;
        col[15] = kept ? d2d : 0.0;
    }
    wave_tree16(col);
    const unsigned long long mk = __builtin_amdgcn_ballot_w64(kept), mf = __builtin_amdgcn_ballot_w64(fell_back);
    double extra = 0.0;
    if constexpr (FULL) extra = wave_tree2(d2d, have ? sqrt(d2d) : 0.0);
    if ((lane & 15) == 0) {
        const int q = lane >> 4;
#pragma unroll
        for (int j = 0; j < 4; ++j) shw_row[1 + 4 * q + j] = col[j];
        if (lane == 0) {
            shw_row[0] = (double)__builtin_popcountll(mk);
            shw_row[NSUMS - 1] = (double)__builtin_popcountll(mf);
            shw_row[17] = extra;
        }
        if (lane == 32) shw_row[18] = extra;
    }
}

template <bool FMA, bool BATCH, int WQ, int NT, int U, bool FIRST = false>
__device__ __forceinline__ void serve_walkers(const PassArgs& a, const GridPairDev& pr, const int32_t* __restrict__ cs,
                                              const float4* __restrict__ sorted, int w, int nwalk, int2 (*rowq)[WQ],
                                              unsigned (*s_ent)[PASS_BS], const unsigned short* s_wl) {
#define KSS_STAMP(k) do { if (a.stamps && threadIdx.x == 0) a.stamps[(size_t)blockIdx.x * 16 + (k)] = __builtin_amdgcn_s_memrealtime(); } while (0)
    enum { WK_X, WK_Y, WK_Z, WK_IDX, WK_D2, WK_R, WK_POS, WK_FL = WK_POS, WK_COLS };
    const GridParams& gp = pr.gp;
    const int lane = threadIdx.x & 63;
    const bool row16 = 16 * nwalk <= NT, row8 = BATCH && !row16 && 8 * nwalk <= NT, rows = row16 || row8;
    const int L = row16 ? 16 : row8 ? 8 : 4 * nwalk <= WQ ? 4 : 1;
    const int nserve = rows ? NT : (WQ < NT ? WQ : NT);
    for (int rb = 0; rb < nwalk; rb += nserve / L)
    if ((int)threadIdx.x < nserve && (int)(threadIdx.x & ~63u) < (nwalk - rb) * L) {
        const int sub = (int)threadIdx.x & (L - 1);
        const int wj = rb + (L == 16 ? (int)threadIdx.x >> 4 : L == 8 ? (int)threadIdx.x >> 3 : L == 4 ? (int)threadIdx.x >> 2 : (int)threadIdx.x);
        const bool wk = wj < nwalk;
        const unsigned rowmask = L == 1 ? 0x1ffu : sub == 0 ? 0x105u : sub == 1 ? 0x050u : sub == 2 ? 0x082u : 0x028u;
        float wx = 0.f, wy = 0.f, wz = 0.f, wrho = __builtin_inff(), bnew = 0.f;
        unsigned long long wkey = ~0ull;
        int wpos = -1, owner = 0, evl = 0, rfin = 0;
        bool done = true, wfell = false;
        if (wk) {
            owner = (int)s_wl[wj];
            wx = __uint_as_float(s_ent[WK_X][owner]); wy = __uint_as_float(s_ent[WK_Y][owner]); wz = __uint_as_float(s_ent[WK_Z][owner]);
            wkey = ((unsigned long long)s_ent[WK_D2][owner] << 32) | (unsigned long long)s_ent[WK_IDX][owner];
            wpos = (int)s_ent[WK_POS][owner];
            wrho = __uint_as_float(s_ent[WK_R][owner]);
            done = false;
        }
        if (wk) {
            const int cx = cell_coord(wx, gp.ox, gp.inv_h, gp.gx), cy = cell_coord(wy, gp.oy, gp.inv_h, gp.gy),
                      cz = cell_coord(wz, gp.oz, gp.inv_h, gp.gz);
            KSS_STAMP(5);
            float m1, m2;
            if (row16) row_walk<FMA, U, false>(gp, cs, sorted, wx, wy, wz, cx, cy, cz, wrho, sub < 9 ? sub : -1, -1, wkey, wpos, m1, m2);
            else if (BATCH && row8) row_walk<FMA, U, true>(gp, cs, sorted, wx, wy, wz, cx, cy, cz, wrho, sub, sub == 0 ? 8 : -1, wkey, wpos, m1, m2);
            else if (FIRST && L == 1) evl = block_walk_first<FMA, WQ, U>(gp, cs, sorted, wx, wy, wz, cx, cy, cz, wrho, a.skin, rowq, wkey, wpos, m1, m2);
            else evl = block_walk<FMA, WQ, U>(gp, cs, sorted, wx, wy, wz, cx, cy, cz, wrho, rowmask, rowq, wkey, wpos, m1, m2);
            if (L > 1) {
#define KSS_GROUP_MERGE(X)                                                                                                          \
do {                                                                                                                            \
    const unsigned olo = (unsigned)X((int)(unsigned)wkey), ohi = (unsigned)X((int)(unsigned)(wkey >> 32));                      \
    const int opos = X(wpos);                                                                                                   \
    const float o1 = __int_as_float(X(__float_as_int(m1))), o2 = __int_as_float(X(__float_as_int(m2)));                         \
    const unsigned long long okey = ((unsigned long long)ohi << 32) | olo;                                                      \
    if (okey < wkey) { wkey = okey; wpos = opos; }                                                                            \
    m2 = fminf(fmaxf(m1, o1), fminf(m2, o2));                                \
    m1 = fminf(m1, o1);                                                                                                         \
} while (0)
                auto x1 = [](int v) { return __builtin_amdgcn_update_dpp(0, v, 0xb1, 0xf, 0xf, false); };
                auto x2 = [](int v) { return __builtin_amdgcn_update_dpp(0, v, 0x4e, 0xf, 0xf, false); };
                auto x4 = [](int v) { const int r = __builtin_amdgcn_update_dpp(v, v, 0x104, 0xf, 0x5, false); return __builtin_amdgcn_update_dpp(r, v, 0x114, 0xf, 0xa, false); };
                auto x8 = [](int v) { return __builtin_amdgcn_update_dpp(0, v, 0x128, 0xf, 0xf, false); };
                KSS_GROUP_MERGE(x1);
                KSS_GROUP_MERGE(x2);
                if (L >= 8) KSS_GROUP_MERGE(x4);
                if (L == 16) KSS_GROUP_MERGE(x8);
#undef KSS_GROUP_MERGE
            }
            float face2 = __builtin_inff();
            for (int r = 1; r <= gp.rcap; ++r) {
                if (r > 1) {
                    const int wd = 2 * r + 1;
                    const int x0 = max(cx - r, 0), x1 = min(cx + r, gp.gx - 1);
                    for (int t = 0; t < wd * wd; ++t) {
                        const int dz = t / wd - r, dy = t % wd - r;
                        const int z = cz + dz, y = cy + dy;
                        if (z < 0 || z >= gp.gz || y < 0 || y >= gp.gy) continue;
                        const int row = (z * gp.gy + y) * gp.gx;
                        if (dz == -r || dz == r || dy == -r || dy == r) {
                            scan_range<FMA>(sorted, cs[row + x0], cs[row + x1 + 1], wx, wy, wz, wkey, wpos);
                        } else {
                            if (cx - r >= 0) scan_range<FMA>(sorted, cs[row + cx - r], cs[row + cx - r + 1], wx, wy, wz, wkey, wpos);
                            if (cx + r < gp.gx) scan_range<FMA>(sorted, cs[row + cx + r], cs[row + cx + r + 1], wx, wy, wz, wkey, wpos);
                        }
                    }
                }
                const float best = __uint_as_float((unsigned)(wkey >> 32));
                float b = __builtin_inff();
                if (cx - r > 0) b = fminf(b, wx - (gp.ox + (float)(cx - r) * gp.h));
                if (cx + r < gp.gx - 1) b = fminf(b, (gp.ox + (float)(cx + r + 1) * gp.h) - wx);
                if (cy - r > 0) b = fminf(b, wy - (gp.oy + (float)(cy - r) * gp.h));
                if (cy + r < gp.gy - 1) b = fminf(b, (gp.oy + (float)(cy + r + 1) * gp.h) - wy);
                if (cz - r > 0) b = fminf(b, wz - (gp.oz + (float)(cz - r) * gp.h));
                if (cz + r < gp.gz - 1) b = fminf(b, (gp.oz + (float)(cz + r + 1) * gp.h) - wz);
                const float bs = b - gp.eps;
                if (b == __builtin_inff()) done = true;
                else if (bs > 0.f && best < bs * bs * 0.999999f) { done = true; face2 = bs * bs; }
                if (done) { rfin = r; break; }
            }
            if (done && rfin == 1 && wkey != ~0ull)
                bnew = fminf(__builtin_amdgcn_sqrtf(fminf(fminf(m2, wrho), face2) * 0.99999f) * 0.999999f, 1e30f);
        }
        if constexpr (BATCH) {
            if (__builtin_amdgcn_ballot_w64(!done) != 0ull) {
                const float4* __restrict__ tp = a.tgt4 + pr.tgt_base;
                for (int j = 0; j < pr.tgt_n; ++j) {
                    const float4 q = tp[j];
                    const float dx = wx - q.x, dy = wy - q.y, dz = wz - q.z;
                    float d;
                    if constexpr (FMA) d = __builtin_fmaf(dx, dx, __builtin_fmaf(dy, dy, dz * dz));
                    else d = (dx * dx + dy * dy) + dz * dz;
                    const unsigned long long kk = ((unsigned long long)__float_as_uint(d) << 32) | (unsigned long long)(unsigned)j;
                    if (!done && kk < wkey) { wkey = kk; wpos = -1; }
                }
                wfell = !done;
                done = true;
            }
        }
        if (wk && sub == 0) {
            bool whave = false;
            float4 ww = make_float4(0.f, 0.f, 0.f, 0.f);
            const int io = pr.src_base + (w - pr.row_base) * PASS_BS + owner;
            if (done) {
                whave = wkey != ~0ull;
                if (whave) ww = wpos >= 0 ? sorted[wpos] : wpos == -2 ? a.nn_win[io] : a.tgt4[pr.tgt_base + (int)(unsigned)(wkey & 0xffffffffull)];
            } else {
                a.keys[io] = ~0ull;
                const int ls = atomicAdd(a.list_count, 1);
                a.list[ls] = io;
                wfell = true;
            }
            a.nn_win[io] = make_float4(ww.x, ww.y, ww.z, __uint_as_float(whave ? (unsigned)wkey : ~0u));
            a.nn_state[io] = make_float2(wfell ? 0.f : bnew, 0.f);
            s_ent[WK_X][owner] = __float_as_uint(ww.x); s_ent[WK_Y][owner] = __float_as_uint(ww.y); s_ent[WK_Z][owner] = __float_as_uint(ww.z);
            s_ent[WK_IDX][owner] = (unsigned)wkey; s_ent[WK_D2][owner] = (unsigned)(wkey >> 32);
            s_ent[WK_FL][owner] = (whave ? 1u : 0u) | (wfell ? 2u : 0u);
            s_ent[WK_R][owner] = __float_as_uint(wfell ? 0.f : bnew);
        }
        KSS_STAMP(8);
        if (a.stamps) {
            int evs = evl, mx = evl;
#pragma unroll
            for (int m = 32; m > 0; m >>= 1) { evs += __shfl_xor(evs, m, 64); mx = max(mx, __shfl_xor(mx, m, 64)); }
            if (lane == 0) {
                atomicAdd(&a.stamps[(size_t)blockIdx.x * 16 + 10], (unsigned long long)evs);
                atomicAdd(&a.stamps[(size_t)blockIdx.x * 16 + 11], (unsigned long long)(((mx + 7) / 8) * 8 * 64));
            }
        }
    }
#undef KSS_STAMP
}

#ifndef KSS_SINGLE_WAVES
#define KSS_SINGLE_WAVES 1
#endif
template <bool FMA, bool FULL, bool SEARCH, bool CHAIN, bool FIRST = false>
__global__ __launch_bounds__(PASS_BS, KSS_SINGLE_WAVES) void grid_pass_kernel(const PassArgs a) {
    static_assert(!CHAIN || SEARCH, "chained launches: search passes");
    static_assert(!FIRST || (SEARCH && !CHAIN), "the first pass: a plain search launch");
#define KSS_STAMP(k) do { if (a.stamps && threadIdx.x == 0) a.stamps[(size_t)blockIdx.x * 16 + (k)] = __builtin_amdgcn_s_memrealtime(); } while (0)
    KSS_STAMP(0);
    constexpr int BS = PASS_BS;
    const int per_xcd = (int)gridDim.x / 8;
    const int w = ((int)blockIdx.x % 8) * per_xcd + (int)blockIdx.x / 8;
    if (w >= a.total_rows) return;
    const GridPairDev pr = a.pair0;
    PairState ps = a.ps0;
    const GridParams& gp = pr.gp;
    const int32_t* __restrict__ cs = a.cell_start + pr.cell_base;
    const float4* __restrict__ sorted = a.sorted;
    constexpr int WQ = FIRST ? BS : 256;
    __shared__ int2 rowq[9][WQ];
    __shared__ double shw[BS / 64][NSUMS];
    __shared__ int s_last;
    __shared__ int sh_ps[16];
    __shared__ int s_nwalk;
    __shared__ unsigned s_ent[7][BS];
    __shared__ unsigned short s_wl[BS];
    enum { WK_X, WK_Y, WK_Z, WK_IDX, WK_D2, WK_R, WK_POS, WK_FL = WK_POS, WK_COLS };
    static_assert(sizeof(PairState) == 64, "the gated launch reads the transform record as 16 dwords");
    double (*shf)[NSUMS] = reinterpret_cast<double (*)[NSUMS]>(&rowq[0][0]);
    static_assert(sizeof(double) * PASS_FG * NSUMS <= sizeof(int2) * 9 * WQ, "shf must fit inside rowq");

    const int local = (w - pr.row_base) * BS + (int)threadIdx.x;
    const bool valid = local < pr.src_n;
    const int i = pr.src_base + local;
    const int lane = threadIdx.x & 63, wave = threadIdx.x >> 6;
    bool have = false, fell_back = false;
    float qx = 0.f, qy = 0.f, qz = 0.f, d2 = 0.f;
    float4 win = make_float4(0.f, 0.f, 0.f, 0.f);
    float4 p = make_float4(0.f, 0.f, 0.f, 0.f), prevp = make_float4(0.f, 0.f, 0.f, __uint_as_float(~0u));
    float2 st = make_float2(0.f, 0.f);
    if (valid) {
        p = SEARCH ? a.src_in[i] : a.src_out[i];
        if (!SEARCH || a.use_prev) { prevp = a.nn_win[i]; st = a.nn_state[i]; }
    }
    for (int step = 0;; ++step) {
    const bool last_step = !CHAIN || step + 1 >= a.chain_len;
    const unsigned long long seq_k = a.seq + (unsigned long long)step;
    const int gate_k = a.gate_seq != 0 ? a.gate_seq + step : 0;
    unsigned int* const gate_ptr = a.gate_dev + 32 * ((a.gate_slot + step) & 1);
    float4* const src_out_k = (step & 1) ? a.src_alt : a.src_out;
    const bool last_known = a.chained == 2 && ps.pad[0] > 0;
    const bool chained_k = step > 0 || a.chained == 1 || last_known;
    const bool has_prev = __float_as_uint(prevp.w) != ~0u;
    if constexpr (SEARCH) {
        __syncthreads();
        if (threadIdx.x == 0) s_nwalk = 0;
        __syncthreads();
    }
    KSS_STAMP(13);
    if constexpr (SEARCH) {
        if (gate_k != 0) {
            typedef unsigned int u32x4 __attribute__((ext_vector_type(4)));
            if (a.state && w == 0 && threadIdx.x < 16) {
                const int* w32 = reinterpret_cast<const int*>(a.state);
                int v = 0, n = 0;
                bool ok = true;
                for (;;) {
                    v = __hip_atomic_load(w32 + threadIdx.x, __ATOMIC_RELAXED, __HIP_MEMORY_SCOPE_SYSTEM);
                    if (__shfl(v, 15, 64) == gate_k) break;
                    __builtin_amdgcn_s_sleep(1);
                    if (++n > a.gate_polls / 2) { ok = false; break; }
                }
                if (ok) {
                    const int g = threadIdx.x;
                    const int w0 = __shfl(v, min(3 * g, 15), 64), w1 = __shfl(v, min(3 * g + 1, 15), 64), w2 = __shfl(v, min(3 * g + 2, 15), 64);
                    if (g < 5) {
                        u32x4 o;
                        o.x = (unsigned)w0; o.y = (unsigned)w1; o.z = (unsigned)w2; o.w = (unsigned)gate_k + kss_mix3(o.x, o.y, o.z);
                        unsigned int* dst = gate_ptr + 4 * g;
                        asm volatile("global_store_dwordx4 %0, %1, off sc1" ::"v"(dst), "v"(o) : "memory");
                    }
                }
            }
            if (threadIdx.x < 8) {
                const unsigned int* src = gate_ptr + 4 * min((int)threadIdx.x, 4);
                u32x4 v;
                int n = 0;
                bool ok = true;
                for (;;) {
                    asm volatile("global_load_dwordx4 %0, %1, off sc0 sc1\n\ts_waitcnt vmcnt(0)" : "=&v"(v) : "v"(src) : "memory");
                    if (__builtin_amdgcn_ballot_w64(v.w - kss_mix3(v.x, v.y, v.z) == (unsigned)gate_k) == 0xffull) break;
                    __builtin_amdgcn_s_sleep(1);
                    if (++n > a.gate_polls) { ok = false; break; }
                }
                if (threadIdx.x < 5) { sh_ps[3 * threadIdx.x] = (int)v.x; sh_ps[3 * threadIdx.x + 1] = (int)v.y; sh_ps[3 * threadIdx.x + 2] = (int)v.z; }
// ... 643 lines not shown
```

kss-icp_amd/csrc/kss_internal.hpp:

```cpp
#pragma once
#include <hip/hip_runtime.h>

#include <algorithm>
#include <cfloat>
#include <cmath>
#include <cstdint>
#include <functional>
#include <string>
#include <vector>

#include "../../include/kssicp.h"
#include "kss_handover.hpp"
#include "kss_host_math.hpp"

namespace kss {

struct alignas(16) PairState {
    float m[12];
    int32_t active;
    int32_t apply;
    int32_t pad[2];
};

struct alignas(16) NNWork {
    int32_t pair;
    int32_t src_begin;
    int32_t src_count;
    int32_t tgt_begin;
    int32_t tgt_count;
    int32_t tgt_pair_base;
    int32_t key_begin;
    int32_t write_src;
};

struct alignas(16) RedWork {
    int32_t pair;
    int32_t src_begin;
    int32_t src_count;
    int32_t key_begin;
    int32_t key_stride;
    int32_t n_split;
    int32_t tgt_pair_base;
    int32_t partial_index;
};

struct PairRed {
    int32_t first;
    int32_t count;
};

struct GridParams {
    float ox, oy, oz;
    float h, inv_h;
    float eps;
    int32_t gx, gy, gz;
    int32_t rcap;
};

struct alignas(16) GridPairDev {
    GridParams gp;
    int32_t cell_base;
    int32_t tgt_base, tgt_n;
    int32_t src_base, src_n;
    int32_t tgt_pad;
    int32_t row_base, n_rows;
    int32_t sorted_base;
};

struct PackSeg {
    int64_t in_off;
    int64_t out_base;
    int64_t n;
};

struct alignas(16) Granule { unsigned long long bits, seq; };

struct PassArgs {
    const float4* src_in; float4* src_out;
    const int32_t* cell_start;
    const float4* sorted;
    const float4* tgt4;
    float4* nn_win;
    float2* nn_state;
    int32_t chained;
    const float4* src_last0; const float4* src_last1;
    float skin;
    unsigned long long* keys;
    int32_t* list; int32_t* list_count;
    const GridPairDev* pairs;
    const int32_t* row_pair;
    const PairState* state;
    GridPairDev pair0; PairState ps0;
    int32_t total_rows, use_prev;
    int32_t gate_polls;
    int32_t chain_len, gate_slot;
    float4* src_alt;
    int32_t gate_seq;
    int32_t defer_pairs;
    unsigned int* gate_dev;
    double max_d2;
    Granule* rows;
    unsigned long long* pub; unsigned long long seq;
    int32_t* idx_out; float* d2_out;
    unsigned long long* stamps;
    int32_t test_torn;
};

constexpr int RES_THREADS = 1024;
constexpr int RES_SMAX = 10;
constexpr int RES_NQ = 640;
constexpr int RES_QW = 4;
constexpr int RES_G = 4;
constexpr int RES_LDS_MAX = 160 * 1024 - 256;
struct ResArgs {
    const GridPairDev* pairs;
    const int32_t* cell_start;
    const float4* sorted;
    const float4* src0;
    unsigned int* gate;
    unsigned long long* pub;
    unsigned long long seq0;
    unsigned int stamp0;
    double max_d2;
    float skin;
    int32_t gate_polls, max_passes, full_always;
    int32_t ntc, tabc;
    int32_t* idx_out; float* d2_out;
    unsigned long long* exit_flags;
    unsigned int exit_tag;
    const int32_t* perm;
    int32_t first_pass, split_at;
    float4* st_pos; unsigned int* st_wc;
    unsigned long long* stamps;
};
size_t resident_lds_bytes(int ntc, int tabc);
int launch_resident(hipStream_t st, bool fma, int npairs, const ResArgs& a, std::string& err);

struct OctBox {
    double min[3], max[3];
    double res;
    int32_t depth;
};

constexpr int NN_TILE = 256;
constexpr int NN_SUB = 32;
constexpr int NN_THREADS = 256;

inline void oct_first_point(OctBox& b, const float* p) {
    const float minValue = FLT_EPSILON;
    for (int k = 0; k < 3; ++k) { b.min[k] = p[k] - b.res / 2; b.max[k] = p[k] + b.res / 2; }
    unsigned maxv = 2;
    for (int k = 0; k < 3; ++k) maxv = std::max(maxv, (unsigned)std::ceil((b.max[k] - b.min[k] - minValue) / b.res));
    b.depth = (int)std::ceil(std::log2((double)maxv) - minValue);
    const double side = (double)(1u << b.depth) * b.res;
    for (int k = 0; k < 3; ++k) {
        const double over = (side - (b.max[k] - b.min[k])) / 2.0;
        if (over > minValue) { b.min[k] -= over; b.max[k] += over; }
    }
}
inline bool oct_adopt(OctBox& b, const float* p) {
    const float minValue = FLT_EPSILON;
    for (;;) {
        bool up[3], any = false;
        for (int k = 0; k < 3; ++k) { up[k] = p[k] >= b.max[k]; any = any || up[k] || p[k] < b.min[k]; }
        if (!any) return true;
        if (b.depth >= 21) return false;
        double side = (double)(1u << b.depth) * b.res;
        for (int k = 0; k < 3; ++k) if (!up[k]) b.min[k] -= side;
        ++b.depth;
        side = (double)(1u << b.depth) * b.res - minValue;
        for (int k = 0; k < 3; ++k) b.max[k] = b.min[k] + side;
    }
}

void launch_pack_f3_to_f4(hipStream_t st, const float* d_in, int64_t n, float4* d_out, int64_t n_pad, bool sentinel);
void launch_pack_f64_to_f4(hipStream_t st, const double* d_in, int64_t n, float4* d_out, int64_t n_pad, bool sentinel);
void launch_empty(hipStream_t st);
int pack_pair_bbox_rows(int64_t nt_pad);
void launch_pack_pair(hipStream_t st, int dtype, const void* d_tgt, int64_t nt, float4* d_tgt_out, int64_t nt_pad, float* d_bbox_partial,
                      const void* d_src, int64_t ns, float4* d_src_out, unsigned int* d_box_host, unsigned box_tag);
void launch_pack_batch(hipStream_t st, const void* d_in, int dtype, const PackSeg* d_seg, int nseg, int64_t total_out, float4* d_out);

void launch_nn_sweep(hipStream_t st, int S, bool fma, const NNWork* d_work, int n_work,
                     const PairState* d_state, const float4* d_src_in, float4* d_src_out,
                     const float4* d_tgt4, unsigned long long* d_keys);

void launch_nn_sweep_list(hipStream_t st, int S, bool fma, const NNWork* d_work, int n_work,
                          const PairState* d_state, float4* d_src_cur, const float4* d_tgt4,
                          unsigned long long* d_keys, const int32_t* d_list, const int32_t* d_count);
void launch_grid_build_pair(hipStream_t st, const float4* d_tgt, int nt, float4* d_src, int ns, const GridParams& gp, int32_t* d_counts,
                            int32_t* d_slot, int32_t* d_start, int32_t* d_block_sums, float4* d_sorted, float4* d_tmp);
size_t scan_scratch_bytes(int n);
int grid_pass_blocks(int total_rows);
void launch_grid_pass(hipStream_t st, bool fma, bool full, bool batch, bool search, const PassArgs& a);
void launch_gridb_bbox(hipStream_t st, const float4* d_tgt, const GridPairDev* d_pairs, int npairs, float* d_bbox);
void launch_gridb_build_targets(hipStream_t st, const float4* d_tgt, int total_tgt_pad, const GridPairDev* d_pairs, int npairs,
                                int total_cells, int32_t* d_counts, int32_t* d_start, int32_t* d_block_sums, float4* d_sorted);
void launch_gridb_sort_sources(hipStream_t st, const float4* d_src, int total_src, const GridPairDev* d_pairs, int npairs,
                               int total_cells, int32_t* d_counts, int32_t* d_start, int32_t* d_block_sums, float4* d_tmp, float4* d_out);
int gridb_lds_max_cells(bool half);
bool launch_gridb_build_lds(hipStream_t st, const float4* d_tgt4, float4* d_src, float4* d_tmp, const GridPairDev* d_pairs, int npairs,
                            int32_t* d_cell_start, float4* d_sorted, int max_cells, bool half);
void launch_grid_stats(hipStream_t st, const float4* d_src, int ns, const GridParams& gp, const int32_t* d_cell_start,
                       unsigned long long* d_out );

void launch_corr_reduce(hipStream_t st, const RedWork* d_work, int n_work, const PairState* d_state,
                        const float4* d_src, const float4* d_tgt4, const unsigned long long* d_keys,
                        double max_d2, double* d_partials, int32_t* d_idx_out, float* d_d2_out, int index_in_w);
void launch_corr_reduce_publish(hipStream_t st, const RedWork* d_work, int n_work, const PairState* d_state,
                                const float4* d_src, const float4* d_tgt4, const unsigned long long* d_keys,
                                double max_d2, Granule* d_rows, int32_t* d_idx_out, float* d_d2_out, int index_in_w,
                                const PairRed* d_pair_red, unsigned long long* d_pub, unsigned long long seq);
size_t cand_pass_lds_bytes(int nt_pad);
int cand_pass_blocks_per_pair(int64_t ns);
bool launch_cand_pass(hipStream_t st, bool fma, int npairs, const PairState* d_state, const float4* d_src_in, float4* d_src_out, const float4* d_tgt,
                      int nt_pad, int ns, double max_d2, Granule* d_rows, unsigned long long* d_pub, unsigned long long seq,
                      int32_t* d_idx_out, float* d_d2_out);
constexpr int CAND_TPW = 4;
struct CandArgs {
    const float4* src0;
    const float4* tgt;
    int32_t nt_pad, ns;
    int32_t bpp, wpp, tpw;
    double max_d2;
    Granule* rows;
    const unsigned int* gate;
    unsigned long long* pub;
    unsigned long long seq0;
    unsigned int stamp0;
    int32_t gate_polls, max_passes;
    int32_t* idx_out; float* d2_out;
    unsigned long long* exit_flags;
    unsigned long long* stamps;
};
int cand_resident_capacity(bool fma, int nt_pad);
int launch_cand_resident(hipStream_t st, bool fma, int npairs, const CandArgs& a, std::string& err);
void launch_corr_reduce_idx(hipStream_t st, const float* d_src3, const float* d_tgt3, const int32_t* d_idx,
                            int64_t n, double max_d2, double* d_partials, int n_blocks);
void launch_finalize_sums(hipStream_t st, const PairRed* d_pairs, int n_pairs, const double* d_partials,
                          double* d_out );

void launch_preshape_pair(hipStream_t st, const void* const d_xyz[2], const int64_t n[2], int dtype, Granule* d_rows,
                          double* d_cent, unsigned long long* d_pub, unsigned long long seq_sum, unsigned long long seq);
void launch_sum_columns(hipStream_t st, const double* d_partials, int n_rows, int n_cols, double* d_out);
void launch_row_sums(hipStream_t st, const double* d_partials, int n_rows, int n_cols, double scale, double* d_out);

void launch_pose_apply(hipStream_t st, const double* d_in, int64_t n, const kss_pose& pose,
                       const double cs[6], double* d_out);
constexpr int POSE_MANY = 32;
void launch_pose_apply_many(hipStream_t st, const double* d_in, int64_t n, const kss_pose& pose, const double (*cs)[6], int count, double* d_out);
void launch_transform_apply_f64(hipStream_t st, const float T[16], const double* d_in, int64_t n, double* d_out);

void launch_transform_apply_f32(hipStream_t st, const float T[16], const float* d_in, int64_t n, float* d_out);
int octree_voxels_device(hipStream_t st, const float* d_pts, int n, const OctBox& box, float* d_cen, int* m_out, std::string& err,
                         const std::function<void*(int, size_t)>& scratch);
void launch_fps(hipStream_t st, const double* d_xyz, int n, int m, double* d_mind, int32_t* d_idx, double* d_out);

int rot_search_grain(int64_t ns, int64_t nt, int g);
void launch_rot_search(hipStream_t st, const double* d_src, int64_t ns, const float4* d_tgt4, int64_t nt_pad ,
                       const double* d_cs , int g, double* d_partials, int n_src_blocks , int nth);

int knn_plan_splits(int nq, int nt_pad, int k, size_t* scratch_bytes);
void launch_knn_sweep(hipStream_t st, const float4* d_qry, int nq, const float4* d_tgt, int nt_pad, int k, int32_t* d_idx, float* d_d2,
                      int n_split, void* d_scratch);
void launch_normals(hipStream_t st, const float4* d_pts, int n, const int32_t* d_knn, int k, double* d_normals);

int preshape_blocks(int64_t n);
inline int stream_blocks(int64_t n) {
    return (int)std::max<int64_t>(1, std::min<int64_t>(2048, (n + 255) / 256));
}

static_assert(P2L_NSUMS == KSS_P2L_NSUMS, "kss_host_math.hpp and include/kssicp.h disagree");
struct PairSrc {
    const float* src3; const float4* src4; const int32_t* perm; const int32_t* idx; const float* d2; const float* sn;
    double max_d2;
};
struct PairArgs {
    PairSrc s;
    const float* tgt; const float* nrm;
    int64_t n, nt;
    double* rows; float* keys;
};
int p2l_rows_blocks(int64_t n);
template <class M>
void launch_pair_rows(hipStream_t st, const PairArgs& a, const M& m);
void launch_p2l_perm(hipStream_t st, const float4* d_src, int64_t n, int32_t* d_perm);
void launch_p2l_final(hipStream_t st, const double* d_rows, int nrows, double* d_out);

constexpr int VMAP_NSTAT = 10;
constexpr int64_t VMAP_MAX_CELLS = 1ll << 26;
static_assert(VMAP_NSTAT == KSS_VMAP_NSTAT, "kss_internal.hpp and include/kssicp.h disagree");
struct VmapDev {
    const int32_t* cell; const double* rec;
    float lo[3]; float inv;
    int dims[3];
};
struct VmapMove { float m[12] = {1, 0, 0, 0, 0, 1, 0, 0, 0, 0, 1, 0}; };
struct VmapBuilt {
    int32_t* cell = nullptr; double* rec = nullptr; int64_t* lin = nullptr;
    int64_t mapped = 0, nvox = 0;
    int dims[3] = {0, 0, 0};
    float lo[3] = {0, 0, 0}, inv = 0;
};
int vmap_build(hipStream_t st, const float* d_tgt, const float* d_nrm, int64_t nt, float inv, VmapBuilt& out);
void vmap_free(VmapBuilt& b);
struct GicpRot;
void launch_vgicp_rows(hipStream_t st, const PairArgs& a, const VmapDev& v, const VmapMove* T, const float* d_in, float* d_out, const GicpRot& Rn,
                       double e);
void launch_scan(hipStream_t st, int32_t* d_counts, int ncells, int32_t* d_start, int32_t* d_scratch, bool clear);

struct alignas(16) TrimState {
    unsigned prefix, pad;
    long long rank, m, k;
    double cut;
    long long kept;
};
constexpr int TRIM_NSTATE = 4;
__host__ __device__ inline long long trim_rank_of(long long m, double overlap) {
    if (m == 0) return 0;
    const double x = overlap * (double)m;
    const long long k = (long long)ceil(x);
    return k < 1 ? 1 : k;
}
int trim_hist_blocks(int64_t n);
size_t trim_rows_bytes(int64_t n);
void launch_trim_select(hipStream_t st, const float* d_d2, int64_t n, double max_d2, double overlap, unsigned* d_rows,
                        TrimState* d_state, double* d_info);
void launch_trim_point_final(hipStream_t st, const double* d_rows, int nrows, double* d_out);
void launch_sim_final(hipStream_t st, const double* d_rows, int nrows, double* d_out);
void launch_f64_to_f32(hipStream_t st, const double* d_in, int64_t n, float* d_out);

struct RobustScale {
    int loss = 0, autoscale = 0;
    double c2 = 0.0, K = 0.0, min2 = 0.0;
};
void launch_robust_plane_final(hipStream_t st, const double* d_rows, int nrows, const RobustScale& rs, const TrimState* d_sel, double* d_out,
                               double* d_info);
void launch_robust_point_final(hipStream_t st, const double* d_rows, int nrows, const RobustScale& rs, const TrimState* d_sel, double* d_out,
                               double* d_info);


struct alignas(16) PairbDesc {
    int64_t src_base, ns;
    int64_t tgt_off, nt;
    double overlap;
    int32_t row_base, nrows;
};
struct PairPass {
    float r[9];
    int32_t align;
    double e;
};
static_assert(sizeof(PairPass) == 48, "the host and the device table share this layout");
struct PairbArgs {
    PairSrc s;
    const float* tgt; const float* nrm;
    const PairbDesc* desc; const int32_t* row_pair; const PairState* state; const RobustScale* rs; TrimState* ts; const PairPass* pass;
    double* rows; float* keys;
};
template <class M>
void launch_pairb_rows(hipStream_t st, int total_rows, const PairbArgs& a);
void launch_pairb_select(hipStream_t st, const float* d_d2, const PairbDesc* d_desc, int npairs, const PairState* d_state, double max_d2,
                         TrimState* d_ts, double* d_info);
void launch_pairb_robust_select(hipStream_t st, int npairs, const PairbArgs& a, const float* d_keys, double bound);
void launch_pairb_final(hipStream_t st, bool plane, int npairs, const PairbArgs& a, double* d_out, bool sim = false);
void launch_pairb_robust_final(hipStream_t st, bool plane, int npairs, const PairbArgs& a, double* d_out, double* d_info);

struct O2oArgs {
    const int32_t* idx; const float* d2;
    const PairbDesc* desc; const int32_t* row_pair; const PairState* state;
    double max_d2;
    unsigned long long* table; unsigned* counters;
    int32_t* idx_out; float* d2_out;
    double* info_m;
};
size_t o2o_table_bytes(int64_t total_tgt, int npairs);
int launch_o2o(hipStream_t st, int total_rows, int64_t total_tgt, int npairs, const O2oArgs& a);

struct RecipGrid {
    float ox, oy, oz, inv_h;
    int32_t gx, gy, gz;
};
constexpr int RECIP_BOX_BLOCKS = 256;
constexpr int RECIP_GMAX = 64;
constexpr int RECIP_CELLS = 32768;
struct alignas(16) RecipPairDev {
    RecipGrid g;
    int32_t cell_base;
};
static_assert(sizeof(RecipPairDev) == 32, "the host and the device table share this layout");
struct RecipArgs {
    PairSrc s;
    const float* tgt;
    const PairbDesc* desc; const int32_t* row_pair; const PairState* state; const RecipPairDev* grids;
    void* work; int64_t total_tgt; int32_t npairs;
    float4* sorted;
    int32_t* idx_out; float* d2_out;
    double* info_mu;
    PairbDesc lone_desc; RecipPairDev lone_grid;
};
__host__ __device__ inline int64_t recip_cells(const RecipGrid& g) { return (int64_t)g.gx * g.gy * g.gz; }
size_t recip_work_bytes(int64_t total_tgt, int npairs, int64_t total_cells);
__host__ __device__ inline unsigned* recip_counters(void* work, int64_t total_tgt) { return (unsigned*)((unsigned long long*)work + total_tgt); }
void launch_recip_bbox(hipStream_t st, const float* d_tgt, const PairbDesc* d_desc, const PairbDesc& lone, int npairs, int split, float* d_box);
int launch_recip(hipStream_t st, int total_rows, int64_t total_cells, const RecipArgs& a, bool nn_fma);

constexpr int64_t PAIRB_INDEX_MAX = 0x7fff0000ll;
inline bool pairb_desc_of(const int64_t* off, const int64_t* tgt_off, int nseg, std::vector<PairbDesc>& desc, int64_t& total_rows) {
    desc.resize((size_t)nseg);
    total_rows = 0;
    for (int i = 0; i < nseg; ++i) {
        PairbDesc& d = desc[i];
        d.src_base = off[i]; d.ns = off[i + 1] - off[i];
        d.tgt_off = tgt_off[i]; d.nt = tgt_off[i + 1] - tgt_off[i]; d.overlap = 1.0;
        d.row_base = (int32_t)total_rows; d.nrows = stream_blocks(d.ns);
        total_rows += d.nrows;
        if (total_rows > PAIRB_INDEX_MAX || tgt_off[i + 1] - tgt_off[0] > PAIRB_INDEX_MAX) return false;
    }
    return true;
}
inline RecipGrid recip_grid_of(const float mn[3], const float mx[3], int64_t n) {
    RecipGrid g = {0.0f, 0.0f, 0.0f, 0.0f, 1, 1, 1};
    double ext[3], vol = 1.0, emax = 0.0;
    int k = 0;
    for (int a = 0; a < 3; ++a) {
        if (!std::isfinite(mn[a]) || !std::isfinite(mx[a]) || mx[a] < mn[a]) return g;
        ext[a] = (double)mx[a] - (double)mn[a];
        if (ext[a] > 0.0) { ++k; vol *= ext[a]; emax = std::max(emax, ext[a]); }
    }
    if (k == 0) return g;
    const double want = (double)std::max<int64_t>(1, std::min<int64_t>(n / 2, RECIP_CELLS));
    const float h = (float)std::max(std::pow(vol / want, 1.0 / k), emax / (RECIP_GMAX - 0.5));
    const float inv_h = 1.0f / h;
    if (!(h > 0.0f) || !std::isfinite(inv_h) || !std::isfinite(h)) return g;
    g.ox = mn[0]; g.oy = mn[1]; g.oz = mn[2];
    g.inv_h = inv_h;
    int* gg[3] = {&g.gx, &g.gy, &g.gz};
    for (int a = 0; a < 3; ++a)
        *gg[a] = ext[a] > 0.0 ? (int)std::max(1.0, std::min((double)RECIP_GMAX, std::floor(ext[a] / (double)h) + 1.0)) : 1;
    return g;
}
inline int64_t recip_grids_of(const float* box, int split, const std::vector<PairbDesc>& desc, std::vector<RecipPairDev>& grids) {
    grids.resize(desc.size());
    int64_t cells = 0;
    for (size_t p = 0; p < desc.size(); ++p) {
        float mn[3] = {INFINITY, INFINITY, INFINITY}, mx[3] = {-INFINITY, -INFINITY, -INFINITY};
        for (int b = 0; b < split; ++b)
            for (int k = 0; k < 3; ++k) {
                mn[k] = std::fmin(mn[k], box[(p * split + b) * 6 + k]);
                mx[k] = std::fmax(mx[k], box[(p * split + b) * 6 + 3 + k]);
            }
        grids[p].g = recip_grid_of(mn, mx, desc[p].ns);
        grids[p].cell_base = (int32_t)cells;
        cells += recip_cells(grids[p].g);
        if (cells > PAIRB_INDEX_MAX) return -1;
    }
    return cells;
}

int aivs_device(hipStream_t st, const double* d_xyz, int n, int point_num, std::vector<int32_t>& out_idx, std::string& err,
                const std::function<void*(size_t)>& scratch);

}
```

Measured before the change: 84120 iterations/s.

## Compute grid parameters on device and launch cell-list build without host round-trip

The grid-parameter choice (bbox reduction and cell sizing) moves into the first build kernel. All build kernels are launched at once using a worst-case cell-count bound, and each reads the device-published GridBuildRec. The host then only spins on a mapped pinned record to learn the chosen grid, instead of waiting for the bbox before launching the build. This overlaps launch latency with the bbox reduction. In exchange it over-allocates and zeroes counters for the bound grid, and it adds a host spin-wait with a stream-sync fallback.

```diff
diff --git a/kss-icp_amd/csrc/kss_api.hip b/kss-icp_amd/csrc/kss_api.hip
--- a/kss-icp_amd/csrc/kss_api.hip
+++ b/kss-icp_amd/csrc/kss_api.hip
@@ -65,7 +65,7 @@
     DevBuf* bufs[] = {&c->tgt4, &c->src0, &c->cur[0], &c->cur[1], &c->keys, &c->partials, &c->sums, &c->nn_work,
                       &c->red_work, &c->pair_red, &c->state, &c->cs, &c->scratch_a, &c->scratch_b, &c->scratch_c,
                       &c->stage_src, &c->stage_tgt, &c->stage_idx, &c->stage_d2, &c->stage_out, &c->g_counts, &c->g_slot, &c->g_start,
-                      &c->g_cursor, &c->g_bsums, &c->g_sorted, &c->g_list, &c->g_count, &c->g_bbox, &c->g_partials, &c->g_start2, &c->g_pairs, &c->g_stamps, &c->g_pos, &c->g_nnst, &c->res_pos, &c->res_wc, &c->res_perm, &c->pack_seg, &c->reg_s, &c->reg_t, &c->reg_p, &c->reg_all, &c->reg_f, &c->reg_g, &c->oct_pts, &c->oct_cen, &c->oct_a, &c->oct_b, &c->oct_tmp, &c->pre_partials, &c->pre_state, &c->g_rowpair, &c->g_gate, &c->p2l_idx, &c->p2l_d2, &c->p2l_perm, &c->p2l_rows, &c->p2l_nrm, &c->p2l_n64, &c->trim_rows, &c->trim_state, &c->rob_keys, &c->gicp_snrm, &c->pb_desc, &c->pb_rowpair, &c->pb_nrm, &c->pb_rscale, &c->pb_snrm, &c->pb_gicp, &c->o2o_table, &c->o2o_idx, &c->o2o_d2, &c->recip_sorted, &c->recip_box, &c->recip_grids, &c->gate_bar, &c->res_gate, &c->bar_state};
+                      &c->g_cursor, &c->g_bsums, &c->g_sorted, &c->g_list, &c->g_count, &c->g_bbox, &c->g_partials, &c->g_start2, &c->g_pairs, &c->g_stamps, &c->g_pos, &c->g_nnst, &c->res_pos, &c->res_wc, &c->res_perm, &c->pack_seg, &c->reg_s, &c->reg_t, &c->reg_p, &c->reg_all, &c->reg_f, &c->reg_g, &c->oct_pts, &c->oct_cen, &c->oct_a, &c->oct_b, &c->oct_tmp, &c->pre_partials, &c->pre_state, &c->g_rowpair, &c->g_gate, &c->p2l_idx, &c->p2l_d2, &c->p2l_perm, &c->p2l_rows, &c->p2l_nrm, &c->p2l_n64, &c->trim_rows, &c->trim_state, &c->rob_keys, &c->gicp_snrm, &c->pb_desc, &c->pb_rowpair, &c->pb_nrm, &c->pb_rscale, &c->pb_snrm, &c->pb_gicp, &c->o2o_table, &c->o2o_idx, &c->o2o_d2, &c->recip_sorted, &c->recip_box, &c->recip_grids, &c->gate_bar, &c->res_gate, &c->bar_state, &c->g_rec};
     for (DevBuf* b : bufs)
         if (b->p) hipFree(b->p);
     if (c->h_sums) hipHostFree(c->h_sums);
@@ -73,6 +73,7 @@
     if (c->h_p2l) hipHostFree(c->h_p2l);
     if (c->h_gicp) hipHostFree(c->h_gicp);
     if (c->h_box) hipHostFree(c->h_box);
+    if (c->h_rec) hipHostFree(c->h_rec);
     if (c->h_xf) hipHostFree(c->h_xf);
     if (c->h_state) hipHostFree(c->h_state);
     for (kss_vmap* m : c->vmaps) { vmap_free(m->b); delete m; }
@@ -123,6 +124,32 @@
     if (!c || !out) return KSS_ERR_ARG;
     out[0] = c->evals_sum; out[1] = c->evals_launches;
     c->evals_sum = 0.0; c->evals_launches = 0.0;
+    return KSS_OK;
+}
+
+int kss_debug_choose_cells(const float mn[3], const float mx[3], int64_t nt, float hscale, void* out) {
+    if (!mn || !mx || !out || nt < 1) return KSS_ERR_ARG;
+    GridParams gp;
+    choose_cells(mn, mx, nt, hscale > 0.f ? hscale : grid_hscale_setting(), gp);
+    std::memcpy(out, &gp, sizeof gp);
+    return KSS_OK;
+}
+int kss_debug_grid_bound(int64_t nt, float hscale) { return nt < 1 ? KSS_ERR_ARG : grid_cells_bound(nt, hscale > 0.f ? hscale : grid_hscale_setting()); }
+int kss_debug_grid_rec(kss_ctx* c, void* out) {
+    if (!c || !out) return KSS_ERR_ARG;
+    if (!c->build_dev_ran) return 0;
+    HIPCHK(c, hipStreamSynchronize(c->stream));
+    HIPCHK(c, hipMemcpy(out, c->g_rec.p, sizeof(GridBuildRec), hipMemcpyDeviceToHost));
+    return 1;
+}
+int kss_debug_grid_lists(kss_ctx* c, int32_t* starts, int64_t nstarts, float* sorted, int64_t nt, float* src, int64_t ns) {
+    if (!c || !starts || !sorted || !src) return KSS_ERR_ARG;
+    const int64_t cells = (int64_t)c->grid_stats[1] * (int64_t)c->grid_stats[2] * (int64_t)c->grid_stats[3];
+    if (cells < 1 || nstarts != 2 * cells + 1 || nt != (int64_t)c->grid_stats[7] || ns != (int64_t)c->grid_stats[6]) return KSS_ERR_ARG;
+    HIPCHK(c, hipStreamSynchronize(c->stream));
+    HIPCHK(c, hipMemcpy(starts, (const int32_t*)c->g_start.p + 1, (size_t)nstarts * sizeof(int32_t), hipMemcpyDeviceToHost));
+    HIPCHK(c, hipMemcpy(sorted, c->g_sorted.p, (size_t)nt * sizeof(float4), hipMemcpyDeviceToHost));
+    HIPCHK(c, hipMemcpy(src, c->src0.p, (size_t)ns * sizeof(float4), hipMemcpyDeviceToHost));
     return KSS_OK;
 }
 
diff --git a/kss-icp_amd/csrc/kss_ctx.hpp b/kss-icp_amd/csrc/kss_ctx.hpp
--- a/kss-icp_amd/csrc/kss_ctx.hpp
+++ b/kss-icp_amd/csrc/kss_ctx.hpp
@@ -71,6 +71,9 @@
     std::vector<float> h_bbox;
     unsigned int* h_box = nullptr; unsigned int* h_box_dev = nullptr; size_t h_box_bytes = 0;
     unsigned box_tag = 0; int box_rows = 0;
+    DevBuf g_rec;
+    unsigned int* h_rec = nullptr; unsigned int* h_rec_dev = nullptr;
+    bool build_dev = false, build_dev_ran = false;
     double evals_sum = 0.0, evals_launches = 0.0;
     void* h_sums = nullptr;  size_t h_sums_cap = 0;
     void* h_sums_dev = nullptr;
@@ -246,6 +249,7 @@
 namespace kss {
 int icp_run_dev(kss_ctx* c, const void* d_src, const int64_t* src_off, const void* d_tgt, const int64_t* tgt_off,
                 int npairs, bool shared_target, int dtype, const kss_icp_params* p, kss_icp_result* results);
+float grid_hscale_setting();
 int nn_generic_dev(kss_ctx* c, const void* d_src, int64_t ns, const void* d_tgt, int64_t nt, int dtype,
                    int32_t* d_idx, float* d_d2, double sums_out[NSUMS]);
 struct PairMode {
diff --git a/kss-icp_amd/csrc/kss_engine.hip b/kss-icp_amd/csrc/kss_engine.hip
--- a/kss-icp_amd/csrc/kss_engine.hip
+++ b/kss-icp_amd/csrc/kss_engine.hip
@@ -218,6 +218,22 @@
     return KSS_OK;
 }
 
+static bool build_device_ready(kss_ctx* c, int nbb) {
+    const char* e = getenv("KSS_BUILD_DEVICE");
+    if ((e && atoi(e) == 0) || nbb > 1024) return false;
+    if (!c->h_rec) {
+        void* hp = nullptr; void* dp = nullptr;
+        if (hipHostMalloc(&hp, 128, hipHostMallocMapped) != hipSuccess || hipHostGetDevicePointer(&dp, hp, 0) != hipSuccess) {
+            if (hp) hipHostFree(hp);
+            (void)hipGetLastError();
+            return false;
+        }
+        std::memset(hp, 0, 128);
+        c->h_rec = (unsigned int*)hp; c->h_rec_dev = (unsigned int*)dp;
+    }
+    return ensure(c, c->g_rec, 128) == KSS_OK;
+}
+
 static int pack_clouds(kss_ctx* c, const IcpPlan& pl, const void* d_src, const int64_t* src_off, const void* d_tgt,
                 const int64_t* tgt_off, int dtype) {
     const size_t esz = dtype == KSS_F64 ? sizeof(double) : sizeof(float);
@@ -227,7 +243,8 @@
         KCHK(ensure(c, c->g_bbox, (size_t)nbb * 6 * sizeof(float)));
         static const bool box_host = !(getenv("KSS_BBOX_HOST") && atoi(getenv("KSS_BBOX_HOST")) == 0);
         c->box_tag = 0; c->box_rows = 0;
-        if (box_host && nbb <= 8192) {
+        c->build_dev = build_device_ready(c, nbb);
+        if (!c->build_dev && box_host && nbb <= 8192) {
             const size_t want = (size_t)nbb * 32;
             if (want > c->h_box_bytes) {
                 if (c->h_box) { HIPCHK(c, hipStreamSynchronize(c->stream)); HIPCHK(c, hipHostFree(c->h_box)); c->h_box = nullptr; c->h_box_dev = nullptr; c->h_box_bytes = 0; }
@@ -277,32 +294,15 @@
     return KSS_OK;
 }
 
-static void choose_cells(const float mn[3], const float mx[3], int64_t nt, GridParams& gp) {
-    const float ext[3] = {mx[0] - mn[0], mx[1] - mn[1], mx[2] - mn[2]};
-    const float emax = std::max(ext[0], std::max(ext[1], ext[2]));
+static float grid_hscale() {
     float hscale = 2.0f;
     if (const char* e = getenv("KSS_GRID_HSCALE")) { const float v = (float)atof(e); if (v > 0.05f && v < 50.f) hscale = v; }
-    float h = emax * hscale * std::sqrt(3.0f / (float)nt);
-    h = std::max(h, emax / 255.5f);
-    if (!(h > 0.f)) h = 1.f;
-    gp.ox = mn[0]; gp.oy = mn[1]; gp.oz = mn[2];
-    gp.h = h; gp.inv_h = 1.0f / h;
-    gp.gx = std::max(1, std::min(256, (int)std::floor(ext[0] / h) + 1));
-    gp.gy = std::max(1, std::min(256, (int)std::floor(ext[1] / h) + 1));
-    gp.gz = std::max(1, std::min(256, (int)std::floor(ext[2] / h) + 1));
-    const float mag = std::max(std::max(std::fabs(mn[0]), std::fabs(mx[0])), std::max(std::max(std::fabs(mn[1]), std::fabs(mx[1])), std::max(std::fabs(mn[2]), std::fabs(mx[2]))));
-    gp.eps = 2e-6f * (mag + emax) + 1e-30f;
-    gp.rcap = 4;
-}
-
-static int grid_setup(kss_ctx* c, IcpPlan& pl) {
-    if (!pl.grid) return KSS_OK;
-    const PairGeom& g = pl.g[0];
-    const int nt = (int)g.nt, ns = (int)g.ns;
-    const int nbb = pack_pair_bbox_rows(g.tgt_pad);
-    const float4* tgt = (const float4*)c->tgt4.p + g.tgt_base;
-    ProfScope ps(c, KSS_K_GRID_BUILD);
-    float mn[3] = {INFINITY, INFINITY, INFINITY}, mx[3] = {-INFINITY, -INFINITY, -INFINITY};
+    return hscale;
+}
+float grid_hscale_setting() { return grid_hscale(); }
+
+static int grid_box_host(kss_ctx* c, int nbb, float mn[3], float mx[3]) {
+    for (int k = 0; k < 3; ++k) { mn[k] = INFINITY; mx[k] = -INFINITY; }
     bool have_box = false;
     if (c->box_tag != 0 && c->box_rows == nbb) {
         const unsigned long long* hq = (const unsigned long long*)c->h_box;
@@ -332,12 +332,10 @@
         for (int b = 0; b < nbb; ++b)
             for (int k = 0; k < 3; ++k) { mn[k] = std::min(mn[k], hb[(size_t)b * 6 + k]); mx[k] = std::max(mx[k], hb[(size_t)b * 6 + 3 + k]); }
     }
-    if (!(std::isfinite(mn[0]) && std::isfinite(mn[1]) && std::isfinite(mn[2]) && std::isfinite(mx[0]) && std::isfinite(mx[1]) && std::isfinite(mx[2])))
-        return set_err(c, KSS_ERR_ARG, "non-finite target coordinates");
-    GridParams gp;
-    choose_cells(mn, mx, nt, gp);
-    pl.gp = gp;
-    const size_t ncells = (size_t)gp.gx * gp.gy * gp.gz;
+    return KSS_OK;
+}
+
+static int grid_ensure(kss_ctx* c, size_t ncells, int nt, int ns) {
     KCHK(ensure_zeroed(c, c->g_counts, 2 * ncells * sizeof(int32_t)));
     KCHK(ensure(c, c->g_slot, ((size_t)nt + (size_t)ns) * sizeof(int32_t)));
     KCHK(ensure(c, c->g_start, (2 * ncells + 8) * sizeof(int32_t)));
@@ -347,25 +345,100 @@
     KCHK(ensure(c, c->g_pos, (size_t)ns * sizeof(float4)));
     c->nn_have = false;
     KCHK(ensure(c, c->g_nnst, (size_t)ns * sizeof(float2)));
-    KCHK(ensure_zeroed(c, c->g_count, 64));
-    if (getenv("KSS_COUNTS_CHECK")) {
+    return ensure_zeroed(c, c->g_count, 64);
+}
+
+static int grid_counts_check(kss_ctx* c, const GridParams& gp) {
+    if (!getenv("KSS_COUNTS_CHECK")) return KSS_OK;
+    const size_t ncells = (size_t)gp.gx * gp.gy * gp.gz;
+    HIPCHK(c, hipStreamSynchronize(c->stream));
+    std::vector<int32_t> h(2 * ncells);
+    HIPCHK(c, hipMemcpy(h.data(), c->g_counts.p, h.size() * sizeof(int32_t), hipMemcpyDeviceToHost));
+    size_t bad = 0, first = 0;
+    for (size_t k = 0; k < h.size(); ++k)
+        if (h[k] != 0) { if (!bad) first = k; ++bad; }
+    if (bad) {
+        std::fprintf(stderr, "[kss] counts check: %zu cells x 2 (%d x %d x %d), buffer %zu bytes, %zu non-zero counters, first at %zu = %d\n", ncells,
+                     gp.gx, gp.gy, gp.gz, c->g_counts.cap, bad, first, h[first]);
+        return set_err(c, KSS_ERR_HIP, "cell counters not zero at rest");
+    }
+    return KSS_OK;
+}
+
+static int grid_rec_collect(kss_ctx* c, unsigned tag, GridBuildRec& rec) {
+    const unsigned long long* hq = (const unsigned long long*)c->h_rec;
+    unsigned w[18];
+    auto look = [&]() {
+        for (int g = 0; g < 6; ++g) {
+            const unsigned long long w0 = __atomic_load_n(&hq[2 * g], __ATOMIC_ACQUIRE), w1 = __atomic_load_n(&hq[2 * g + 1], __ATOMIC_ACQUIRE);
+            const unsigned x = (unsigned)w0, y = (unsigned)(w0 >> 32), z = (unsigned)w1;
+            if ((unsigned)(w1 >> 32) - kss_mix3(x, y, z) != tag) return false;
+            w[3 * g] = x; w[3 * g + 1] = y; w[3 * g + 2] = z;
+        }
+        return true;
+    };
+    const auto t0 = std::chrono::steady_clock::now();
+    bool got = false;
+    for (long spin = 0; !(got = look()); ++spin) {
+        __builtin_ia32_pause();
+        if ((spin & 4095) == 4095 && std::chrono::duration<double, std::milli>(std::chrono::steady_clock::now() - t0).count() > 20.0) break;
+    }
+    if (!got) {
         HIPCHK(c, hipStreamSynchronize(c->stream));
-        std::vector<int32_t> h(2 * ncells);
-        HIPCHK(c, hipMemcpy(h.data(), c->g_counts.p, h.size() * sizeof(int32_t), hipMemcpyDeviceToHost));
-        size_t bad = 0, first = 0;
-        for (size_t k = 0; k < h.size(); ++k)
-            if (h[k] != 0) { if (!bad) first = k; ++bad; }
-        if (bad) {
-            std::fprintf(stderr, "[kss] counts check: %zu cells x 2 (%d x %d x %d), buffer %zu bytes, %zu non-zero counters, first at %zu = %d\n", ncells,
-                         gp.gx, gp.gy, gp.gz, c->g_counts.cap, bad, first, h[first]);
-            return set_err(c, KSS_ERR_HIP, "cell counters not zero at rest");
-        }
-    }
+        if (!look()) return set_err(c, KSS_ERR_HIP, "the cell-list build finished without publishing its grid");
+    }
+    std::memcpy(&rec, w, sizeof rec);
+    return KSS_OK;
+}
+
+static int grid_setup(kss_ctx* c, IcpPlan& pl) {
+    if (!pl.grid) return KSS_OK;
+    const PairGeom& g = pl.g[0];
+    const int nt = (int)g.nt, ns = (int)g.ns;
+    const int nbb = pack_pair_bbox_rows(g.tgt_pad);
+    const float4* tgt = (const float4*)c->tgt4.p + g.tgt_base;
+    const float hscale = grid_hscale();
+    ProfScope ps(c, KSS_K_GRID_BUILD);
+    float mn[3], mx[3];
+    GridParams gp;
+    bool built = false, have_box = false;
+    c->build_dev_ran = false;
+    if (c->build_dev) {
+        const int gcap = grid_cells_bound(nt, hscale);
+        KCHK(grid_ensure(c, (size_t)gcap * gcap * gcap, nt, ns));
+        unsigned tag = (unsigned)(++c->seq);
+        if (tag == 0) tag = (unsigned)(++c->seq);
+        launch_grid_build_pair_dev(c->stream, tgt, nt, (float4*)c->src0.p + g.src_base, ns, (const float*)c->g_bbox.p, nbb, hscale, gcap,
+                                   (GridBuildRec*)c->g_rec.p, c->h_rec_dev, tag, (int32_t*)c->g_counts.p, (int32_t*)c->g_slot.p,
+                                   (int32_t*)c->g_start.p + 1, (int32_t*)c->g_bsums.p, (float4*)c->g_sorted.p, (float4*)c->cur[0].p);
+        HIPCHK(c, hipGetLastError());
+        GridBuildRec rec;
+        KCHK(grid_rec_collect(c, tag, rec));
+        if (rec.ok == 0) return set_err(c, KSS_ERR_ARG, "non-finite target coordinates");
+        if (rec.ok == 1) {
+            gp = rec.gp;
+            built = true;
+            c->build_dev_ran = true;
+            KCHK(grid_counts_check(c, gp));
+        } else {
+            for (int k = 0; k < 3; ++k) { mn[k] = rec.mn[k]; mx[k] = rec.mx[k]; }
+            have_box = true;
+        }
+    }
+    if (!built) {
+        if (!have_box) KCHK(grid_box_host(c, nbb, mn, mx));
+        if (!(std::isfinite(mn[0]) && std::isfinite(mn[1]) && std::isfinite(mn[2]) && std::isfinite(mx[0]) && std::isfinite(mx[1]) && std::isfinite(mx[2])))
+            return set_err(c, KSS_ERR_ARG, "non-finite target coordinates");
+        choose_cells(mn, mx, nt, hscale, gp);
+        KCHK(grid_ensure(c, (size_t)gp.gx * gp.gy * gp.gz, nt, ns));
+        KCHK(grid_counts_check(c, gp));
+        launch_grid_build_pair(c->stream, tgt, nt, (float4*)c->src0.p + g.src_base, ns, gp, (int32_t*)c->g_counts.p, (int32_t*)c->g_slot.p,
+                               (int32_t*)c->g_start.p + 1, (int32_t*)c->g_bsums.p, (float4*)c->g_sorted.p, (float4*)c->cur[0].p);
+        HIPCHK(c, hipGetLastError());
+    }
+    pl.gp = gp;
     pl.gpairs[0].gp = gp;
     pl.gpairs[0].cell_base = 0;
-    launch_grid_build_pair(c->stream, tgt, nt, (float4*)c->src0.p + g.src_base, ns, gp, (int32_t*)c->g_counts.p, (int32_t*)c->g_slot.p,
-                           (int32_t*)c->g_start.p + 1, (int32_t*)c->g_bsums.p, (float4*)c->g_sorted.p, (float4*)c->cur[0].p);
-    HIPCHK(c, hipGetLastError());
     c->grid_stats[0] = gp.h; c->grid_stats[1] = gp.gx; c->grid_stats[2] = gp.gy; c->grid_stats[3] = gp.gz;
     if (c->stats_ns != ns || c->stats_nt != nt) { c->grid_stats[4] = 0; c->grid_stats[5] = 0; }
     c->grid_stats[6] = ns; c->grid_stats[7] = nt;
@@ -403,7 +476,7 @@
         const float* b = &hb[(size_t)p * 6];
         for (int k = 0; k < 6; ++k)
             if (!std::isfinite(b[k])) return set_err(c, KSS_ERR_ARG, "non-finite target coordinates");
-        choose_cells(b, b + 3, pl.g[p].nt, hp[p].gp);
+        choose_cells(b, b + 3, pl.g[p].nt, grid_hscale(), hp[p].gp);
         hp[p].cell_base = (int32_t)cells;
         hp[p].sorted_base = (int32_t)sorted_base;
         const int64_t nc = (int64_t)hp[p].gp.gx * hp[p].gp.gy * hp[p].gp.gz;
diff --git a/kss-icp_amd/csrc/kss_grid.hip b/kss-icp_amd/csrc/kss_grid.hip
--- a/kss-icp_amd/csrc/kss_grid.hip
+++ b/kss-icp_amd/csrc/kss_grid.hip
@@ -13,8 +13,8 @@
 
 namespace kss {
 
-__global__ __launch_bounds__(256) void grid_count2_kernel(const float4* __restrict__ tgt, int nt, int nbt, const float4* __restrict__ src, int ns,
-                                                          GridParams gp, int32_t* __restrict__ counts, int32_t* __restrict__ slot) {
+__device__ __forceinline__ void grid_count2_body(const float4* __restrict__ tgt, int nt, int nbt, const float4* __restrict__ src, int ns,
+                                                 const GridParams& gp, int32_t* __restrict__ counts, int32_t* __restrict__ slot) {
     const bool is_src = (int)blockIdx.x >= nbt;
     const int i = ((int)blockIdx.x - (is_src ? nbt : 0)) * 256 + (int)threadIdx.x;
     if (i >= (is_src ? ns : nt)) return;
@@ -23,10 +23,76 @@
               cz = cell_coord(p.z, gp.oz, gp.inv_h, gp.gz);
     slot[(is_src ? nt : 0) + i] = atomicAdd(&counts[(is_src ? gp.gx * gp.gy * gp.gz : 0) + (cz * gp.gy + cy) * gp.gx + cx], 1);
 }
+__global__ __launch_bounds__(256) void grid_count2_kernel(const float4* __restrict__ tgt, int nt, int nbt, const float4* __restrict__ src, int ns,
+                                                          GridParams gp, int32_t* __restrict__ counts, int32_t* __restrict__ slot) {
+    grid_count2_body(tgt, nt, nbt, src, ns, gp, counts, slot);
+}
+
+__device__ __forceinline__ int build_cells(const GridBuildRec* __restrict__ rec) {
+    return rec->ok == 1 ? rec->gp.gx * rec->gp.gy * rec->gp.gz : 0;
+}
+__global__ __launch_bounds__(256) void grid_count2_dev_kernel(const float4* __restrict__ tgt, int nt, int nbt, const float4* __restrict__ src, int ns,
+                                                              const float* __restrict__ bbox, int nbb, float hscale, int gcap,
+                                                              GridBuildRec* __restrict__ rec, unsigned int* __restrict__ rec_host, unsigned tag,
+                                                              int32_t* __restrict__ counts, int32_t* __restrict__ slot) {
+    __shared__ float sh[4][6];
+    __shared__ unsigned sh_rec[18];
+    const float inf = __builtin_inff();
+    float b[6] = {inf, inf, inf, -inf, -inf, -inf};
+    for (int r = (int)threadIdx.x; r < nbb; r += 256)
+#pragma unroll
+        for (int k = 0; k < 3; ++k) { b[k] = fminf(b[k], bbox[r * 6 + k]); b[3 + k] = fmaxf(b[3 + k], bbox[r * 6 + 3 + k]); }
+#pragma unroll
+    for (int off = 32; off > 0; off >>= 1)
+#pragma unroll
+        for (int k = 0; k < 3; ++k) {
+            b[k] = fminf(b[k], __shfl_xor(b[k], off, 64));
+            b[3 + k] = fmaxf(b[3 + k], __shfl_xor(b[3 + k], off, 64));
+        }
+    if ((threadIdx.x & 63) == 0)
+#pragma unroll
+        for (int k = 0; k < 6; ++k) sh[threadIdx.x >> 6][k] = b[k];
+    __syncthreads();
+    GridBuildRec r;
+#pragma unroll
+    for (int k = 0; k < 3; ++k) {
+        r.mn[k] = fminf(fminf(sh[0][k], sh[1][k]), fminf(sh[2][k], sh[3][k]));
+        r.mx[k] = fmaxf(fmaxf(sh[0][3 + k], sh[1][3 + k]), fmaxf(sh[2][3 + k], sh[3][3 + k]));
+    }
+    bool finite = true;
+#pragma unroll
+    for (int k = 0; k < 3; ++k) finite = finite && fabsf(r.mn[k]) < inf && fabsf(r.mx[k]) < inf;
+    r.gp = GridParams{0.f, 0.f, 0.f, 0.f, 0.f, 0.f, 0, 0, 0, 0};
+    r.ok = 0; r.pad = 0;
+    if (finite) {
+        choose_cells(r.mn, r.mx, nt, hscale, r.gp);
+        r.ok = r.gp.gx <= gcap && r.gp.gy <= gcap && r.gp.gz <= gcap ? 1 : 2;
+    }
+    if (blockIdx.x == 0) {
+        if (threadIdx.x == 0) {
+            *rec = r;
+            const unsigned w[18] = {__float_as_uint(r.gp.ox), __float_as_uint(r.gp.oy), __float_as_uint(r.gp.oz), __float_as_uint(r.gp.h),
+                                    __float_as_uint(r.gp.inv_h), __float_as_uint(r.gp.eps), (unsigned)r.gp.gx, (unsigned)r.gp.gy, (unsigned)r.gp.gz,
+                                    (unsigned)r.gp.rcap, __float_as_uint(r.mn[0]), __float_as_uint(r.mn[1]), __float_as_uint(r.mn[2]),
+                                    __float_as_uint(r.mx[0]), __float_as_uint(r.mx[1]), __float_as_uint(r.mx[2]), (unsigned)r.ok, 0u};
+#pragma unroll
+            for (int k = 0; k < 18; ++k) sh_rec[k] = w[k];
+        }
+        __syncthreads();
+        if (threadIdx.x < 6) {
+            u32x4 g;
+            g.x = sh_rec[3 * threadIdx.x]; g.y = sh_rec[3 * threadIdx.x + 1]; g.z = sh_rec[3 * threadIdx.x + 2]; g.w = tag + kss_mix3(g.x, g.y, g.z);
+            unsigned int* dst = rec_host + 4 * threadIdx.x;
+            asm volatile("global_store_dwordx4 %0, %1, off sc0 sc1" ::"v"(dst), "v"(g) : "memory");
+        }
+    }
+    if (r.ok != 1) return;
+    grid_count2_body(tgt, nt, nbt, src, ns, r.gp, counts, slot);
+}
 
 constexpr int SCAN_CHUNK = 4096;
 
-__global__ __launch_bounds__(256) void scan_block_sums_kernel(const int32_t* __restrict__ in, int n, int32_t* __restrict__ block_sums) {
+__device__ __forceinline__ void scan_block_sums_body(const int32_t* __restrict__ in, int n, int32_t* __restrict__ block_sums) {
     __shared__ int sh[4];
     typedef int32_t int4u __attribute__((ext_vector_type(4), aligned(4)));
     const int base = blockIdx.x * SCAN_CHUNK;
@@ -43,8 +109,17 @@
     __syncthreads();
     if (threadIdx.x == 0) block_sums[blockIdx.x] = sh[0] + sh[1] + sh[2] + sh[3];
 }
-
-__global__ __launch_bounds__(1024) void scan_of_block_sums_kernel(int32_t* __restrict__ block_sums, int nb) {
+__global__ __launch_bounds__(256) void scan_block_sums_kernel(const int32_t* __restrict__ in, int n, int32_t* __restrict__ block_sums) {
+    scan_block_sums_body(in, n, block_sums);
+}
+__global__ __launch_bounds__(256) void scan_block_sums_dev_kernel(const int32_t* __restrict__ in, const GridBuildRec* __restrict__ rec,
+                                                                  int32_t* __restrict__ block_sums) {
+    const int n = 2 * build_cells(rec);
+    if ((int)blockIdx.x * SCAN_CHUNK >= n) return;
+    scan_block_sums_body(in, n, block_sums);
+}
+
+__device__ __forceinline__ void scan_of_block_sums_body(int32_t* __restrict__ block_sums, int nb) {
     __shared__ int wave_tot[16];
     const int tid = threadIdx.x, lane = tid & 63, wave = tid >> 6;
     const int per = (nb + 1023) / 1024;
@@ -67,10 +142,13 @@
         run += v;
     }
 }
+__global__ __launch_bounds__(1024) void scan_of_block_sums_kernel(int32_t* __restrict__ block_sums, int nb) { scan_of_block_sums_body(block_sums, nb); }
+__global__ __launch_bounds__(1024) void scan_of_block_sums_dev_kernel(int32_t* __restrict__ block_sums, const GridBuildRec* __restrict__ rec) {
+    scan_of_block_sums_body(block_sums, (2 * build_cells(rec) + SCAN_CHUNK - 1) / SCAN_CHUNK);
+}
 
 template <bool SELF, bool CLEAR>
-__global__ __launch_bounds__(256) void scan_apply_kernel(int32_t* in, int n, const int32_t* __restrict__ block_sums,
-                                                         int32_t* __restrict__ out_start) {
+__device__ __forceinline__ void scan_apply_body(int32_t* in, int n, const int32_t* __restrict__ block_sums, int32_t* __restrict__ out_start) {
     typedef int32_t int4u __attribute__((ext_vector_type(4), aligned(4)));
     __shared__ int sh_tot[4][4];
     __shared__ int sh_off[4];
@@ -125,6 +203,18 @@
         run += (sh_tot[k][0] + sh_tot[k][1]) + (sh_tot[k][2] + sh_tot[k][3]);
     }
 }
+template <bool SELF, bool CLEAR>
+__global__ __launch_bounds__(256) void scan_apply_kernel(int32_t* in, int n, const int32_t* __restrict__ block_sums,
+                                                         int32_t* __restrict__ out_start) {
+    scan_apply_body<SELF, CLEAR>(in, n, block_sums, out_start);
+}
+template <bool SELF>
+__global__ __launch_bounds__(256) void scan_apply_dev_kernel(int32_t* in, const GridBuildRec* __restrict__ rec, const int32_t* __restrict__ block_sums,
+                                                             int32_t* __restrict__ out_start) {
+    const int n = 2 * build_cells(rec);
+    if ((int)blockIdx.x * SCAN_CHUNK >= n) return;
+    scan_apply_body<SELF, true>(in, n, block_sums, out_start);
+}
 
 using BigScanConfig = rocprim::scan_config<256, 64, rocprim::block_load_method::block_load_transpose, rocprim::block_store_method::block_store_transpose,
                                            rocprim::block_scan_algorithm::reduce_then_scan>;
@@ -161,9 +251,9 @@
     }
 }
 
-__global__ __launch_bounds__(256) void grid_scatter2_kernel(const float4* __restrict__ tgt, int nt, int nbt, const float4* __restrict__ src, int ns,
-                                                            GridParams gp, const int32_t* __restrict__ slot, const int32_t* __restrict__ start,
-                                                            float4* __restrict__ sorted, float4* __restrict__ src_tmp) {
+__device__ __forceinline__ void grid_scatter2_body(const float4* __restrict__ tgt, int nt, int nbt, const float4* __restrict__ src, int ns,
+                                                   const GridParams& gp, const int32_t* __restrict__ slot, const int32_t* __restrict__ start,
+                                                   float4* __restrict__ sorted, float4* __restrict__ src_tmp) {
     const bool is_src = (int)blockIdx.x >= nbt;
     const int i = ((int)blockIdx.x - (is_src ? nbt : 0)) * 256 + (int)threadIdx.x;
     if (i >= (is_src ? ns : nt)) return;
@@ -174,6 +264,18 @@
     const int pos = start[cell] + slot[(is_src ? nt : 0) + i] - (is_src ? nt : 0);
     p.w = __int_as_float(i);
     (is_src ? src_tmp : sorted)[pos] = p;
+}
+__global__ __launch_bounds__(256) void grid_scatter2_kernel(const float4* __restrict__ tgt, int nt, int nbt, const float4* __restrict__ src, int ns,
+                                                            GridParams gp, const int32_t* __restrict__ slot, const int32_t* __restrict__ start,
+                                                            float4* __restrict__ sorted, float4* __restrict__ src_tmp) {
+    grid_scatter2_body(tgt, nt, nbt, src, ns, gp, slot, start, sorted, src_tmp);
+}
+__global__ __launch_bounds__(256) void grid_scatter2_dev_kernel(const float4* __restrict__ tgt, int nt, int nbt, const float4* __restrict__ src, int ns,
+                                                                const GridBuildRec* __restrict__ rec, const int32_t* __restrict__ slot,
+                                                                const int32_t* __restrict__ start, float4* __restrict__ sorted,
+                                                                float4* __restrict__ src_tmp) {
+    if (rec->ok != 1) return;
+    grid_scatter2_body(tgt, nt, nbt, src, ns, rec->gp, slot, start, sorted, src_tmp);
 }
 
 template <bool FMA>
@@ -406,9 +508,9 @@
     }
 }
 
-__global__ __launch_bounds__(256) void grid_rank_fix_kernel(const float4* __restrict__ tmp, int n, GridParams gp,
-                                                            const int32_t* __restrict__ start , int shift,
-                                                            float4* __restrict__ out) {
+__device__ __forceinline__ void grid_rank_fix_body(const float4* __restrict__ tmp, int n, const GridParams& gp,
+                                                   const int32_t* __restrict__ start , int shift,
+                                                   float4* __restrict__ out) {
     const int j = blockIdx.x * blockDim.x + threadIdx.x;
     if (j >= n) return;
     const float4 p = tmp[j];
@@ -421,6 +523,17 @@
     for (int k = lo; k < hi; ++k) rank += __float_as_int(tmp[k].w) < me ? 1 : 0;
     out[lo + rank] = p;
 }
+__global__ __launch_bounds__(256) void grid_rank_fix_kernel(const float4* __restrict__ tmp, int n, GridParams gp,
+                                                            const int32_t* __restrict__ start , int shift,
+                                                            float4* __restrict__ out) {
+    grid_rank_fix_body(tmp, n, gp, start, shift, out);
+}
+__global__ __launch_bounds__(256) void grid_rank_fix_dev_kernel(const float4* __restrict__ tmp, int n, const GridBuildRec* __restrict__ rec,
+                                                                const int32_t* __restrict__ start ,
+                                                                int shift, float4* __restrict__ out) {
+    if (rec->ok != 1) return;
+    grid_rank_fix_body(tmp, n, rec->gp, start + build_cells(rec), shift, out);
+}
 
 void launch_grid_build_pair(hipStream_t st, const float4* d_tgt, int nt, float4* d_src, int ns, const GridParams& gp, int32_t* d_counts,
                             int32_t* d_slot, int32_t* d_start, int32_t* d_block_sums, float4* d_sorted, float4* d_tmp) {
@@ -432,6 +545,26 @@
                        (const int32_t*)d_start, d_sorted, d_tmp);
     hipLaunchKernelGGL(grid_rank_fix_kernel, dim3(nbs), dim3(256), 0, st, (const float4*)d_tmp, ns, gp, (const int32_t*)d_start + ncells, nt,
                        d_src);
+}
+
+void launch_grid_build_pair_dev(hipStream_t st, const float4* d_tgt, int nt, float4* d_src, int ns, const float* d_bbox, int nbb, float hscale,
+                                int gcap, GridBuildRec* d_rec, unsigned int* d_rec_host, unsigned tag, int32_t* d_counts, int32_t* d_slot,
+                                int32_t* d_start, int32_t* d_block_sums, float4* d_sorted, float4* d_tmp) {
+    const int nbt = (nt + 255) / 256, nbs = (ns + 255) / 256;
+    const int nb = (2 * gcap * gcap * gcap + SCAN_CHUNK - 1) / SCAN_CHUNK;
+    const GridBuildRec* rec = d_rec;
+    hipLaunchKernelGGL(grid_count2_dev_kernel, dim3(nbt + nbs), dim3(256), 0, st, d_tgt, nt, nbt, (const float4*)d_src, ns, d_bbox, nbb, hscale, gcap,
+                       d_rec, d_rec_host, tag, d_counts, d_slot);
+    hipLaunchKernelGGL(scan_block_sums_dev_kernel, dim3(nb), dim3(256), 0, st, (const int32_t*)d_counts, rec, d_block_sums);
+    if (nb <= 1024) {
+        hipLaunchKernelGGL((scan_apply_dev_kernel<true>), dim3(nb), dim3(256), 0, st, d_counts, rec, (const int32_t*)d_block_sums, d_start);
+    } else {
+        hipLaunchKernelGGL(scan_of_block_sums_dev_kernel, dim3(1), dim3(1024), 0, st, d_block_sums, rec);
+        hipLaunchKernelGGL((scan_apply_dev_kernel<false>), dim3(nb), dim3(256), 0, st, d_counts, rec, (const int32_t*)d_block_sums, d_start);
+    }
+    hipLaunchKernelGGL(grid_scatter2_dev_kernel, dim3(nbt + nbs), dim3(256), 0, st, d_tgt, nt, nbt, (const float4*)d_src, ns, rec, (const int32_t*)d_slot,
+                       (const int32_t*)d_start, d_sorted, d_tmp);
+    hipLaunchKernelGGL(grid_rank_fix_dev_kernel, dim3(nbs), dim3(256), 0, st, (const float4*)d_tmp, ns, rec, (const int32_t*)d_start, nt, d_src);
 }
 
 struct SkipOut {
diff --git a/kss-icp_amd/csrc/kss_internal.hpp b/kss-icp_amd/csrc/kss_internal.hpp
--- a/kss-icp_amd/csrc/kss_internal.hpp
+++ b/kss-icp_amd/csrc/kss_internal.hpp
@@ -56,6 +56,40 @@
     int32_t gx, gy, gz;
     int32_t rcap;
 };
+
+__host__ __device__ inline int grid_axis_cells(float q) {
+    const int g = (int)floorf(q) + 1;
+    return g > 256 ? 256 : g < 1 ? 1 : g;
+}
+__host__ __device__ inline void choose_cells(const float mn[3], const float mx[3], int64_t nt, float hscale, GridParams& gp) {
+#pragma clang fp contract(off)
+    const float ext[3] = {mx[0] - mn[0], mx[1] - mn[1], mx[2] - mn[2]};
+    const float emax = fmaxf(ext[0], fmaxf(ext[1], ext[2]));
+    float h = emax * hscale * sqrtf(3.0f / (float)nt);
+    h = fmaxf(h, emax / 255.5f);
+    if (!(h > 0.f)) h = 1.f;
+    gp.ox = mn[0]; gp.oy = mn[1]; gp.oz = mn[2];
+    gp.h = h; gp.inv_h = 1.0f / h;
+    gp.gx = grid_axis_cells(ext[0] / h);
+    gp.gy = grid_axis_cells(ext[1] / h);
+    gp.gz = grid_axis_cells(ext[2] / h);
+    const float mag = fmaxf(fmaxf(fabsf(mn[0]), fabsf(mx[0])), fmaxf(fmaxf(fabsf(mn[1]), fabsf(mx[1])), fmaxf(fabsf(mn[2]), fabsf(mx[2]))));
+    gp.eps = 2e-6f * (mag + emax) + 1e-30f;
+    gp.rcap = 4;
+}
+
+inline int grid_cells_bound(int64_t nt, float hscale) {
+    const double q = 1.0 / ((double)hscale * std::sqrt(3.0 / (double)std::max<int64_t>(nt, 1)));
+    return (int)std::min(256.0, std::floor(q * (1.0 + 1e-5)) + 1.0);
+}
+
+struct GridBuildRec {
+    GridParams gp;
+    float mn[3], mx[3];
+    int32_t ok;
+    int32_t pad;
+};
+static_assert(sizeof(GridBuildRec) == 18 * sizeof(int32_t), "six granules of three words");
 
 struct alignas(16) GridPairDev {
     GridParams gp;
@@ -190,6 +224,9 @@
                           unsigned long long* d_keys, const int32_t* d_list, const int32_t* d_count);
 void launch_grid_build_pair(hipStream_t st, const float4* d_tgt, int nt, float4* d_src, int ns, const GridParams& gp, int32_t* d_counts,
                             int32_t* d_slot, int32_t* d_start, int32_t* d_block_sums, float4* d_sorted, float4* d_tmp);
+void launch_grid_build_pair_dev(hipStream_t st, const float4* d_tgt, int nt, float4* d_src, int ns, const float* d_bbox, int nbb, float hscale,
+                                int gcap, GridBuildRec* d_rec, unsigned int* d_rec_host, unsigned tag, int32_t* d_counts, int32_t* d_slot,
+                                int32_t* d_start, int32_t* d_block_sums, float4* d_sorted, float4* d_tmp);
 size_t scan_scratch_bytes(int n);
 int grid_pass_blocks(int total_rows);
 void launch_grid_pass(hipStream_t st, bool fma, bool full, bool batch, bool search, const PassArgs& a);
```

Result: no change. 84470 iterations/s, median of 5 (+0.4%).
